# EmbarkStudios/kajiya

Hardware: NVIDIA H100
Metric: gi_rays_per_sec (higher is better)
Workload: dtype f32

## Files before the change

include/kjb_tlas.h:

```cpp
#ifndef KJB_TLAS_H
#define KJB_TLAS_H
#include "kjb.h"
#ifdef __cplusplus
extern "C" {
#endif
int kjb_tlas_download(kjb_context *ctx, uint32_t out_counts[3], int32_t *out_root, void *nodes, void *tris, void *tri_info, int32_t *parent);

#define KJB_TLAS_TRACE_ANY_HIT 1u
#define KJB_TLAS_TRACE_CULL_BACK 2u
#define KJB_TLAS_TRACE_BRUTE_FORCE 4u
int kjb_tlas_trace(kjb_context *ctx, const float *rays, uint32_t n, uint32_t flags, float *out);
#ifdef __cplusplus
}
#endif
#endif
```

kajiya_b200/_abi.py:

```python
import ctypes as C
import numpy as np

FMT = dict(R32_FLOAT=1, RG32_UINT=2, RGBA32_FLOAT=3, RGBA32_UINT=4, RGBA16_FLOAT=5, RG16_FLOAT=6, RGBA8_UNORM=7,
           RGBA8_SNORM=8, R8_UNORM=9, R8_SNORM=10, RGBA16_SNORM=11, A2R10G10B10_UNORM=12, R11G11B10_UFLOAT=13,
           R32_UINT=14, R16_FLOAT=15, RG32_FLOAT=16)
FMT_NAME = {v: k for k, v in FMT.items()}
FMT_NUMPY = {1: (np.float32, 1), 2: (np.uint32, 2), 3: (np.float32, 4), 4: (np.uint32, 4), 5: (np.float16, 4), 6: (np.float16, 2),
             7: (np.uint8, 4), 8: (np.int8, 4), 9: (np.uint8, 1), 10: (np.int8, 1), 11: (np.int16, 4), 12: (np.uint32, 1),
             13: (np.uint32, 1), 14: (np.uint32, 1), 15: (np.float16, 1), 16: (np.float32, 2)}


class Image(C.Structure):
    _fields_ = [("data", C.c_void_p), ("width", C.c_uint32), ("height", C.c_uint32), ("format", C.c_uint32), ("layers", C.c_uint32)]


class Buffer(C.Structure):
    _fields_ = [("data", C.c_void_p), ("size_bytes", C.c_uint64)]


class MeshMaterial(C.Structure):
    _fields_ = [("base_color_mult", C.c_float * 4), ("maps", C.c_uint32 * 4), ("roughness_mult", C.c_float), ("metalness_factor", C.c_float),
                ("emissive", C.c_float * 3), ("flags", C.c_uint32), ("map_transforms", C.c_float * 24)]


class TextureDesc(C.Structure):
    _fields_ = [("texels", C.c_void_p), ("width", C.c_uint32), ("height", C.c_uint32), ("mip_count", C.c_uint32), ("srgb", C.c_uint32)]


class WorldDesc(C.Structure):
    _fields_ = [("render_width", C.c_uint32), ("render_height", C.c_uint32), ("temporal_upscale_width", C.c_uint32), ("temporal_upscale_height", C.c_uint32),
                ("spatial_reuse_pass_count", C.c_uint32), ("use_raytraced_reservoir_visibility", C.c_uint32),
                ("enable_ircache", C.c_uint32), ("enable_rtr", C.c_uint32), ("enable_taa", C.c_uint32), ("tile_y0", C.c_uint32), ("tile_y1", C.c_uint32),
                ("tile_rank", C.c_uint32), ("tile_count", C.c_uint32), ("enable_ssao", C.c_uint32), ("enable_lighting", C.c_uint32), ("hard_sun", C.c_uint32)]


class MeshDesc(C.Structure):
    _fields_ = [("positions", C.c_void_p), ("normals", C.c_void_p), ("uvs", C.c_void_p), ("colors", C.c_void_p), ("material_ids", C.c_void_p),
                ("indices", C.c_void_p), ("vertex_count", C.c_uint32), ("index_count", C.c_uint32), ("materials", C.POINTER(MeshMaterial)),
                ("material_count", C.c_uint32), ("maps", C.POINTER(TextureDesc)), ("map_count", C.c_uint32), ("use_lights", C.c_uint32)]


class WorldFrame(C.Structure):
    _fields_ = [("camera_position", C.c_float * 3), ("camera_rotation", C.c_float * 4), ("vertical_fov_deg", C.c_float), ("near_plane", C.c_float),
                ("sun_direction", C.c_float * 3), ("delta_time_seconds", C.c_float),
                ("host_gbuffer", C.c_void_p), ("host_depth", C.c_void_p), ("host_geometric_normal", C.c_void_p), ("host_velocity", C.c_void_p),
                ("host_result", C.c_void_p), ("capture_slot", C.c_uint32), ("replay_slot", C.c_uint32), ("streaming", C.c_uint32)]


assert C.sizeof(MeshMaterial) == 152


class KjbError(RuntimeError):
    pass


class KjbLib:

    def __init__(self, path):
        self.path = path
        self.dll = C.CDLL(path, mode=C.RTLD_LOCAL)
        d = self.dll
        P = C.c_void_p
        sig = {
            "kjb_abi_version": (C.c_int, []),
            "kjb_backend_name": (C.c_char_p, []),
            "kjb_create": (C.c_int, [C.c_int, C.POINTER(P)]),
            "kjb_destroy": (None, [P]),
            "kjb_sync": (C.c_int, [P]),
            "kjb_last_error": (C.c_char_p, [P]),
            "kjb_launch_count": (C.c_uint64, [P]),
            "kjb_stream": (P, [P]),
            "kjb_format_texel_bytes": (C.c_uint32, [C.c_uint32]),
            "kjb_image_alloc": (C.c_int, [P, C.c_uint32, C.c_uint32, C.c_uint32, C.c_uint32, C.POINTER(Image)]),
            "kjb_image_free": (C.c_int, [P, C.POINTER(Image)]),
            "kjb_image_clear": (C.c_int, [P, C.POINTER(Image)]),
            "kjb_image_upload": (C.c_int, [P, C.POINTER(Image), P]),
            "kjb_image_download": (C.c_int, [P, C.POINTER(Image), P]),
            "kjb_ray_counters": (C.c_int, [P, C.POINTER(C.c_uint64 * 2), C.c_int]),
            "kjb_world_create": (C.c_int, [P, C.POINTER(WorldDesc), C.POINTER(P)]),
            "kjb_world_destroy": (None, [P]),
            "kjb_world_add_mesh": (C.c_int, [P, C.POINTER(MeshDesc), C.POINTER(C.c_uint32)]),
            "kjb_world_add_instance": (C.c_int, [P, C.c_uint32, C.POINTER(C.c_float * 12), C.POINTER(C.c_uint32)]),
            "kjb_world_set_instance_transform": (C.c_int, [P, C.c_uint32, C.POINTER(C.c_float * 12)]),
            "kjb_world_remove_instance": (C.c_int, [P, C.c_uint32]),
            "kjb_world_set_sun_size_multiplier": (C.c_int, [P, C.c_float]),
            "kjb_world_set_sun_color_multiplier": (C.c_int, [P, C.POINTER(C.c_float * 3)]),
            "kjb_world_set_sky_ambient": (C.c_int, [P, C.POINTER(C.c_float * 3)]),
            "kjb_world_set_render_overrides": (C.c_int, [P, C.c_uint32, C.c_float]),
            "kjb_world_set_debug_shading_mode": (C.c_int, [P, C.c_uint32]),
            "kjb_world_reset_reference_accumulation": (C.c_int, [P]),
            "kjb_world_set_instance_emissive_multiplier": (C.c_int, [P, C.c_uint32, C.c_float]),
            "kjb_world_set_blue_noise": (C.c_int, [P, P]),
            "kjb_world_set_spatial_resolve_offsets": (C.c_int, [P, P]),
            "kjb_world_render_frame": (C.c_int, [P, C.POINTER(WorldFrame)]),
            "kjb_world_render_reference": (C.c_int, [P, C.POINTER(WorldFrame), C.c_uint32]),
            "kjb_world_frame_index": (C.c_uint32, [P]),
            "kjb_world_wait": (C.c_int, [P]),
            "kjb_world_get_image": (C.c_int, [P, C.c_char_p, C.POINTER(Image)]),
            "kjb_world_image_names": (C.c_char_p, [P]),
            "kjb_world_last_frame_stats": (C.c_int, [P, C.POINTER(C.c_uint64 * 4)]),
            "kjb_world_set_stop_after": (C.c_int, [P, C.c_char_p]),
            "kjb_world_set_profiling": (C.c_int, [P, C.c_uint32]),
            "kjb_comm_nccl_unique_id": (C.c_int, [P]),
            "kjb_comm_init_nccl": (C.c_int, [P, P, C.c_uint32, C.c_uint32]),
            "kjb_comm_set_callback": (C.c_int, [P, P, P, C.c_uint32, C.c_uint32]),
            "kjb_world_pass_timings": (C.c_char_p, [P]),
            "kjb_set_debug_serial": (C.c_int, [P, C.c_uint32]),
            "kjb_tlas_stats": (C.c_int, [P, C.POINTER(C.c_uint64 * 2)]),
            "kjb_graph_stats": (C.c_int, [P, C.POINTER(C.c_uint64 * 2)]),
            "kjb_graph_select": (C.c_int, [P, C.c_uint32]), "kjb_set_pass_queue": (C.c_int, [P, C.c_uint32]), "kjb_async_passes_supported": (C.c_int, [P]),
            "kjb_world_set_cuda_graph": (C.c_int, [P, C.c_uint32]), "kjb_world_set_async_compute": (C.c_int, [P, C.c_uint32]),
            "kjb_set_option": (C.c_int, [P, C.c_uint32, C.c_uint32]),
            "kjb_timer_record": (C.c_int, [P, C.c_uint32]),
            "kjb_timer_elapsed_ms": (C.c_int, [P, C.c_uint32, C.c_uint32, C.POINTER(C.c_float)]),
        }
        self.missing = []
        for name, (res, args) in sig.items():
            try:
                fn = getattr(d, name)
            except AttributeError:
                self.missing.append(name)
                continue
            fn.restype = res
            fn.argtypes = args
        if self.missing:
            raise KjbError(f"{path} does not export: {self.missing}")
        if d.kjb_abi_version() != 1:
            raise KjbError("ABI version mismatch")
        self.has_tlas_download = hasattr(d, "kjb_tlas_download")
        if self.has_tlas_download:
            d.kjb_tlas_download.restype = C.c_int
            d.kjb_tlas_download.argtypes = [P, C.POINTER(C.c_uint32 * 3), C.POINTER(C.c_int32), P, P, P, P]
        self.has_tlas_trace = hasattr(d, "kjb_tlas_trace")
        if self.has_tlas_trace:
            d.kjb_tlas_trace.restype = C.c_int
            d.kjb_tlas_trace.argtypes = [P, P, C.c_uint32, C.c_uint32, P]

    @property
    def backend(self):
        return self.dll.kjb_backend_name().decode()


def declared_symbols(include_dir):
    import re, os
    names = []
    for h in ("kjb.h", "kjb_world.h"):
        src = open(os.path.join(include_dir, h)).read()
        names += re.findall(r"\b(kjb_[a-z0-9_]+)\s*\(", src)
    return sorted(set(names))
```

kajiya_b200/csrc/kjb_api.cu:

```cuda
#include "kjb_context.h"
#include "kjb_ircache.cuh"
#include "kjb_bvh_build.cuh"
#include "../../include/kjb_tlas.h"
#include <algorithm>

using namespace kjb;

KJB_DEV void box_of_tri(const float3 a, const float3 b, const float3 c, float* out6) {
    out6[0] = kjb_min(a.x, kjb_min(b.x, c.x)); out6[1] = kjb_min(a.y, kjb_min(b.y, c.y)); out6[2] = kjb_min(a.z, kjb_min(b.z, c.z));
    out6[3] = kjb_max(a.x, kjb_max(b.x, c.x)); out6[4] = kjb_max(a.y, kjb_max(b.y, c.y)); out6[5] = kjb_max(a.z, kjb_max(b.z, c.z));
}
KJB_KERNEL(256) k_refit_tris(SceneView sc, BvhTri* tris, float* tri_box, uint32_t slot_count, Rows kjb_rows) {
    const uint32_t s = blockIdx.x * blockDim.x + threadIdx.x;
    if (s >= slot_count) return;
    const uint32_t gid = tris[s].gid;
    if (gid >= sc.tri_count) return;
    const TriInfo ti = sc.tri_info[gid];
    const kjb_instance& inst = sc.instances[ti.instance];
    const kjb_gpu_mesh mesh = sc.meshes[inst.mesh_index];
    float3 wv[3];
    for (int k = 0; k < 3; ++k) {
        const uint32_t idx = vb_u32(sc, mesh.index_offset + (ti.prim * 3 + k) * 4);
        const float* v = reinterpret_cast<const float*>(sc.vertices + mesh.vertex_core_offset + size_t(idx) * 16);
        wv[k] = xform_point(inst.transform, f3(v[0], v[1], v[2]));
    }
    BvhTri t = tris[s];
    t.v0[0] = wv[0].x; t.v0[1] = wv[0].y; t.v0[2] = wv[0].z;
    t.e1[0] = wv[1].x - wv[0].x; t.e1[1] = wv[1].y - wv[0].y; t.e1[2] = wv[1].z - wv[0].z;
    t.e2[0] = wv[2].x - wv[0].x; t.e2[1] = wv[2].y - wv[0].y; t.e2[2] = wv[2].z - wv[0].z;
    tris[s] = t;
    box_of_tri(wv[0], wv[1], wv[2], tri_box + size_t(s) * 6);
}
KJB_KERNEL(256) k_refit_nodes(BvhNode* nodes, const int32_t* parent, uint32_t* count, float* slot_box, const float* tri_box, const uint32_t* node_count, Rows kjb_rows) {
    uint32_t i = blockIdx.x * blockDim.x + threadIdx.x;
    if (i >= *node_count) return;
    uint32_t leaves = 0;
    for (int k = 0; k < 2; ++k) {
        const int32_t ch = nodes[i].child[k];
        if (ch >= 0) continue;
        const uint32_t enc = uint32_t(~ch), first = enc >> 3, n = (enc & 7u) + 1u;
        float b[6] = {3.4e38f, 3.4e38f, 3.4e38f, -3.4e38f, -3.4e38f, -3.4e38f};
        for (uint32_t t = 0; t < n; ++t) for (int a = 0; a < 3; ++a) { b[a] = kjb_min(b[a], tri_box[size_t(first + t) * 6 + a]); b[3 + a] = kjb_max(b[3 + a], tri_box[size_t(first + t) * 6 + 3 + a]); }
        for (int a = 0; a < 6; ++a) slot_box[(size_t(i) * 2 + k) * 6 + a] = b[a];
        write_padded_slot(nodes[i], k, b);
        ++leaves;
    }
    if (leaves == 0) return;
    for (;;) {
#if defined(__CUDA_ARCH__)
        __threadfence();
#endif
        if (atom_add(&count[i], leaves) + leaves < 2u) return;
        const int32_t p = parent[i];
        if (p < 0) return;
        float u[6];
        for (int a = 0; a < 3; ++a) { u[a] = kjb_min(slot_box[(size_t(i) * 2) * 6 + a], slot_box[(size_t(i) * 2 + 1) * 6 + a]); u[3 + a] = kjb_max(slot_box[(size_t(i) * 2) * 6 + 3 + a], slot_box[(size_t(i) * 2 + 1) * 6 + 3 + a]); }
        const uint32_t pi = uint32_t(p >> 1); const int pk = p & 1;
        for (int a = 0; a < 6; ++a) slot_box[(size_t(pi) * 2 + pk) * 6 + a] = u[a];
        write_padded_slot(nodes[pi], pk, u);
        i = pi; leaves = 1;
    }
}

extern "C" {

int kjb_abi_version(void) { return KJB_ABI_VERSION; }
#if defined(KJB_EMU)
const char* kjb_backend_name(void) { return "emu-cpu"; }
#else
#if defined(KJB_FAST)
const char* kjb_backend_name(void) { return "cuda-sm90a-fast"; }
#else
const char* kjb_backend_name(void) { return "cuda-sm90a"; }
#endif
#endif

static thread_local std::string g_create_error;

int kjb_create(int device, kjb_context** out) {
    *out = nullptr;
#if !defined(KJB_EMU)
    int n = 0;
    if (cudaGetDeviceCount(&n) != cudaSuccess || n == 0) { g_create_error = "kjb_create: no CUDA device (this library has no CPU fallback)"; return 1; }
    if (device < 0 || device >= n) { g_create_error = "kjb_create: invalid device ordinal"; return 1; }
    if (cudaSetDevice(device) != cudaSuccess) { g_create_error = "kjb_create: cudaSetDevice failed"; return 1; }
#endif
    kjb_context* c = new kjb_context();
    c->device = device;
#if !defined(KJB_EMU)
    if (cudaStreamCreateWithFlags(&c->compute_stream, cudaStreamNonBlocking) != cudaSuccess) { delete c; g_create_error = "kjb_create: stream creation failed"; return 1; }
    c->stream = c->compute_stream;
#endif
    memset(&c->g, 0, sizeof(c->g));
    c->d_ray_counters = (unsigned long long*)dev_alloc(2 * sizeof(unsigned long long));
    c->g.scene.ray_counters = c->d_ray_counters;
    c->g.scene.root = ~int32_t(0);
    *out = c;
    return 0;
}
void kjb_destroy(kjb_context* c) {
    if (!c) return;
    dev_sync(c);
    dev_free(c->d_vertices); dev_free(c->d_meshes); dev_free(c->d_instances); dev_free(c->d_nodes); dev_free(c->d_tris); dev_free(c->d_tri_info);
    dev_free(c->d_node_parent); dev_free(c->d_refit_count); dev_free(c->d_slot_box); dev_free(c->d_tri_box); dev_free(c->d_bvh_scratch); dev_free(c->d_inst_prefix);
    dev_free(c->d_tex_data); dev_free(c->d_tex_desc); dev_free(c->d_lights); dev_free(c->d_ray_counters); dev_free(c->d_prev_instances); dev_free(c->d_resolve_offsets);
    for (auto& kv : c->ircache_scratch) { const auto& s = kv.second; dev_free(s.claim_rank); dev_free(s.claim_vertex); dev_free(s.life_pending); dev_free(s.scan); dev_free(s.claim_bits); dev_free(s.aux_prev); dev_free(s.entry_vertex); }
#if !defined(KJB_EMU)
    if (c->pinned_staging) cudaFreeHost(c->pinned_staging);
    for (auto& ge : c->graph_execs) if (ge) cudaGraphExecDestroy(ge);
    for (auto& ev : c->queue_events) if (ev) cudaEventDestroy(ev);
    for (auto& st : c->copy_streams) if (st) cudaStreamDestroy(st);
    if (c->compute_stream) cudaStreamDestroy(c->compute_stream);
#endif
    delete c;
}
int kjb_sync(kjb_context* c) {
    if (dev_sync(c)) return c->fail("kjb_sync: stream synchronize failed");
    const char* e = dev_check(c); if (e) return c->fail(std::string("kjb_sync: ") + e);
    return 0;
}
const char* kjb_last_error(kjb_context* c) { return c ? c->last_error.c_str() : g_create_error.c_str(); }
uint64_t kjb_launch_count(kjb_context* c) { return c->launches; }
#if defined(KJB_EMU)
void* kjb_stream(kjb_context* c) { return (void*)c->stream; }
#else
void* kjb_stream(kjb_context* c) { return (void*)c->compute_stream; }
#endif
uint32_t kjb_format_texel_bytes(uint32_t f) { return texel_bytes(f); }

int kjb_image_alloc(kjb_context* c, uint32_t w, uint32_t h, uint32_t layers, uint32_t fmt, kjb_image* out) {
    if (!texel_bytes(fmt) || !w || !h) return c->fail("kjb_image_alloc: bad format or extent");
    out->width = w; out->height = h; out->format = fmt; out->layers = layers ? layers : 1;
    out->data = dev_alloc(image_bytes(*out));
    return out->data ? 0 : c->fail("kjb_image_alloc: out of device memory");
}
static void drop_ircache_scratch(kjb_context* c, const void* p) {
    auto it = c->ircache_scratch.find(p);
    if (it == c->ircache_scratch.end()) return;
    dev_sync(c);
    const auto& s = it->second; dev_free(s.claim_rank); dev_free(s.claim_vertex); dev_free(s.life_pending); dev_free(s.scan); dev_free(s.claim_bits); dev_free(s.aux_prev); dev_free(s.entry_vertex);
    c->ircache_scratch.erase(it);
}
int kjb_image_free(kjb_context* c, kjb_image* img) {
    drop_ircache_scratch(c, img->data);
    dev_free(img->data); img->data = nullptr; return 0;
}
int kjb_image_clear(kjb_context* c, const kjb_image* img) { c->invalidate_positions(); return dev_memset(c, img->data, 0, image_bytes(*img)); }
int kjb_image_fill_u8(kjb_context* c, const kjb_image* img, uint32_t v) { c->invalidate_positions(); return dev_memset(c, img->data, int(v), image_bytes(*img)); }
int kjb_image_copy(kjb_context* c, const kjb_image* dst, const kjb_image* src) { c->invalidate_positions();
    if (image_bytes(*dst) != image_bytes(*src) || dst->format != src->format) return c->fail("kjb_image_copy: extent/format mismatch");
    return dev_d2d(c, dst->data, src->data, image_bytes(*dst));
}
int kjb_image_upload(kjb_context* c, const kjb_image* dst, const void* src) { c->invalidate_positions(); return dev_h2d(c, dst->data, src, image_bytes(*dst)); }
int kjb_image_download(kjb_context* c, const kjb_image* src, void* dst) { return dev_d2h(c, dst, src->data, image_bytes(*src)); }
#if defined(KJB_EMU)
int kjb_image_upload_on(kjb_context* c, uint32_t, const kjb_image* dst, const void* src) { return kjb_image_upload(c, dst, src); }
int kjb_image_download_on(kjb_context* c, uint32_t, const kjb_image* src, void* dst) { return kjb_image_download(c, src, dst); }
int kjb_image_upload_rows_on(kjb_context* c, uint32_t, const kjb_image* dst, const void* src, uint32_t r0, uint32_t n) {
    if (r0 + n > dst->height) return c->fail("kjb_image_upload_rows_on: rows out of range");
    const size_t rb = size_t(dst->width) * texel_bytes(dst->format); c->invalidate_positions(); memcpy((char*)dst->data + rb * r0, (const char*)src + rb * r0, rb * n); return 0; }
int kjb_image_download_rows_on(kjb_context* c, uint32_t, const kjb_image* src, void* dst, uint32_t r0, uint32_t n) {
    if (r0 + n > src->height) return c->fail("kjb_image_download_rows_on: rows out of range");
    const size_t rb = size_t(src->width) * texel_bytes(src->format); memcpy((char*)dst + rb * r0, (const char*)src->data + rb * r0, rb * n); return 0; }
int kjb_event_record(kjb_context*, uint32_t, uint32_t) { return 0; }
int kjb_queue_wait_event(kjb_context*, uint32_t, uint32_t) { return 0; }
int kjb_event_synchronize(kjb_context*, uint32_t) { return 0; }
#else
int kjb_image_upload_on(kjb_context* c, uint32_t q, const kjb_image* dst, const void* src) {
    c->invalidate_positions();
    cudaStream_t st = c->queue(q); if (!st) return c->fail("kjb_image_upload_on: bad queue");
    return cudaMemcpyAsync(dst->data, src, image_bytes(*dst), cudaMemcpyHostToDevice, st) != cudaSuccess ? c->fail("kjb_image_upload_on: copy failed") : 0;
}
int kjb_image_upload_rows_on(kjb_context* c, uint32_t q, const kjb_image* dst, const void* src, uint32_t r0, uint32_t n) {
    if (r0 + n > dst->height || (dst->layers > 1)) return c->fail("kjb_image_upload_rows_on: rows out of range");
    c->invalidate_positions();
    cudaStream_t st = c->queue(q); if (!st) return c->fail("kjb_image_upload_rows_on: bad queue");
    const size_t rb = size_t(dst->width) * texel_bytes(dst->format);
    return cudaMemcpyAsync((char*)dst->data + rb * r0, (const char*)src + rb * r0, rb * n, cudaMemcpyHostToDevice, st) != cudaSuccess ? c->fail("kjb_image_upload_rows_on: copy failed") : 0;
}
int kjb_image_download_rows_on(kjb_context* c, uint32_t q, const kjb_image* src, void* dst, uint32_t r0, uint32_t n) {
    if (r0 + n > src->height || (src->layers > 1)) return c->fail("kjb_image_download_rows_on: rows out of range");
    cudaStream_t st = c->queue(q); if (!st) return c->fail("kjb_image_download_rows_on: bad queue");
    const size_t rb = size_t(src->width) * texel_bytes(src->format);
    return cudaMemcpyAsync((char*)dst + rb * r0, (const char*)src->data + rb * r0, rb * n, cudaMemcpyDeviceToHost, st) != cudaSuccess ? c->fail("kjb_image_download_rows_on: copy failed") : 0;
}
int kjb_image_download_on(kjb_context* c, uint32_t q, const kjb_image* src, void* dst) {
    cudaStream_t st = c->queue(q); if (!st) return c->fail("kjb_image_download_on: bad queue");
    return cudaMemcpyAsync(dst, src->data, image_bytes(*src), cudaMemcpyDeviceToHost, st) != cudaSuccess ? c->fail("kjb_image_download_on: copy failed") : 0;
}
int kjb_event_record(kjb_context* c, uint32_t e, uint32_t q) {
    cudaStream_t st = c->queue(q); if (!st || e >= KJB_MAX_EVENTS) return c->fail("kjb_event_record: bad queue or event");
    if (!c->queue_events[e] && cudaEventCreateWithFlags(&c->queue_events[e], cudaEventDisableTiming) != cudaSuccess) return c->fail("kjb_event_record: cudaEventCreate failed");
    return cudaEventRecord(c->queue_events[e], st) != cudaSuccess ? c->fail("kjb_event_record: record failed") : 0;
}
int kjb_queue_wait_event(kjb_context* c, uint32_t q, uint32_t e) {
    cudaStream_t st = c->queue(q); if (!st || e >= KJB_MAX_EVENTS) return c->fail("kjb_queue_wait_event: bad queue or event");
    if (!c->queue_events[e]) return 0;
    return cudaStreamWaitEvent(st, c->queue_events[e], 0) != cudaSuccess ? c->fail("kjb_queue_wait_event: wait failed") : 0;
}
int kjb_event_synchronize(kjb_context* c, uint32_t e) {
    if (e >= KJB_MAX_EVENTS) return c->fail("kjb_event_synchronize: bad event");
    if (!c->queue_events[e]) return 0;
    return cudaEventSynchronize(c->queue_events[e]) != cudaSuccess ? c->fail("kjb_event_synchronize: failed") : 0;
}
#endif
int kjb_buffer_alloc(kjb_context* c, uint64_t n, kjb_buffer* out) { out->data = dev_alloc(n); out->size_bytes = n; return out->data ? 0 : c->fail("kjb_buffer_alloc: out of device memory"); }
int kjb_buffer_free(kjb_context* c, kjb_buffer* b) { drop_ircache_scratch(c, b->data); dev_free(b->data); b->data = nullptr; return 0; }
int kjb_buffer_upload(kjb_context* c, const kjb_buffer* dst, uint64_t off, const void* src, uint64_t n) { return dev_h2d(c, (char*)dst->data + off, src, n); }
int kjb_buffer_download(kjb_context* c, const kjb_buffer* src, uint64_t off, void* dst, uint64_t n) { return dev_d2h(c, dst, (const char*)src->data + off, n); }

int kjb_scene_set_geometry(kjb_context* c, const void* vb, uint64_t vb_bytes, const kjb_gpu_mesh* meshes, const uint32_t* counts, uint32_t n) {
    dev_sync(c);
    dev_free(c->d_vertices); dev_free(c->d_meshes);
    c->h_vertices.assign((const uint8_t*)vb, (const uint8_t*)vb + vb_bytes);
    c->h_meshes.assign(meshes, meshes + n); c->h_index_counts.assign(counts, counts + n);
    c->d_vertices = (uint8_t*)dev_alloc(vb_bytes); c->d_meshes = (kjb_gpu_mesh*)dev_alloc(n * sizeof(kjb_gpu_mesh));
    if (!c->d_vertices || !c->d_meshes) return c->fail("kjb_scene_set_geometry: out of device memory");
    dev_h2d(c, c->d_vertices, c->h_vertices.data(), vb_bytes); dev_h2d(c, c->d_meshes, c->h_meshes.data(), n * sizeof(kjb_gpu_mesh));
    c->g.scene.vertices = c->d_vertices; c->g.scene.meshes = c->d_meshes;
    c->tlas_valid = false;
    return dev_sync(c);
}
int kjb_scene_set_textures(kjb_context* c, const kjb_texture_desc* t, uint32_t n) {
    dev_sync(c);
    dev_free(c->d_tex_data); dev_free(c->d_tex_desc); c->d_tex_data = nullptr; c->d_tex_desc = nullptr;
    std::vector<uint8_t> data; std::vector<uint4> desc(n);
    for (uint32_t i = 0; i < n; ++i) {
        size_t bytes = 0; for (uint32_t m = 0; m < t[i].mip_count; ++m) bytes += size_t(t[i].width >> m ? t[i].width >> m : 1) * (t[i].height >> m ? t[i].height >> m : 1) * 4;
        desc[i] = u4(uint32_t(data.size()), t[i].width, t[i].height, t[i].mip_count | (t[i].srgb << 16));
        data.insert(data.end(), t[i].texels, t[i].texels + bytes);
        while (data.size() & 15) data.push_back(0);
    }
    c->tex_count = n;
    if (n) {
        c->d_tex_data = (uint8_t*)dev_alloc(data.size()); c->d_tex_desc = (uint4*)dev_alloc(n * sizeof(uint4));
        if (!c->d_tex_data || !c->d_tex_desc) return c->fail("kjb_scene_set_textures: out of device memory");
        dev_h2d(c, c->d_tex_data, data.data(), data.size()); dev_h2d(c, c->d_tex_desc, desc.data(), n * sizeof(uint4));
    }
    c->g.scene.tex_data = c->d_tex_data; c->g.scene.tex_desc = c->d_tex_desc; c->g.scene.tex_count = n;
    return dev_sync(c);
}

static void* staging_slot(kjb_context* c, size_t bytes) {
    if (c->pinned_bytes < bytes) {
#if !defined(KJB_EMU)
        dev_sync(c); if (c->pinned_staging) cudaFreeHost(c->pinned_staging);
        if (cudaMallocHost(&c->pinned_staging, bytes * 4) != cudaSuccess) { c->pinned_staging = nullptr; c->pinned_bytes = 0; return nullptr; }
#else
        free(c->pinned_staging); c->pinned_staging = malloc(bytes * 4);
#endif
        c->pinned_bytes = bytes;
    }
    return (char*)c->pinned_staging + size_t(c->staging_seq++ & 3u) * c->pinned_bytes;
}
static int reserve_tlas(kjb_context* c, uint32_t tris, uint32_t instances) {
    const bool grow_tris = tris > c->bvh_tri_cap || !c->d_bvh_scratch, grow_inst = instances + 1 > c->bvh_inst_cap || !c->d_instances;
    if (!grow_tris && !grow_inst) return 0;
    dev_sync(c);
    if (grow_inst) {
        const uint32_t cap = std::max(instances + 1, c->bvh_inst_cap * 2);
        dev_free(c->d_instances); dev_free(c->d_inst_prefix);
        c->d_instances = (kjb_instance*)dev_alloc(size_t(cap) * sizeof(kjb_instance)); c->d_inst_prefix = (uint32_t*)dev_alloc(size_t(cap + 1) * 4);
        c->bvh_inst_cap = cap;
        if (!c->d_instances || !c->d_inst_prefix) { c->bvh_inst_cap = 0; return c->fail("kjb_rebuild_tlas: out of device memory"); }
    }
    if (grow_tris) {
        const uint32_t cap = std::max(std::max(tris, 1u), c->bvh_tri_cap + c->bvh_tri_cap / 2);
        dev_free(c->d_nodes); dev_free(c->d_tris); dev_free(c->d_tri_info); dev_free(c->d_node_parent); dev_free(c->d_refit_count); dev_free(c->d_slot_box);
        dev_free(c->d_tri_box); dev_free(c->d_bvh_scratch);
        c->d_nodes = (BvhNode*)dev_alloc(size_t(cap) * sizeof(BvhNode)); c->d_tris = (BvhTri*)dev_alloc(size_t(cap) * sizeof(BvhTri));
        c->d_tri_info = (TriInfo*)dev_alloc(size_t(cap + 1) * sizeof(TriInfo)); c->d_node_parent = (int32_t*)dev_alloc(size_t(cap) * 4);
        c->d_refit_count = (uint32_t*)dev_alloc(size_t(cap) * 4); c->d_slot_box = (float*)dev_alloc(size_t(cap) * 12 * sizeof(float));
        c->d_tri_box = (float*)dev_alloc(size_t(cap) * 6 * sizeof(float)); c->d_bvh_scratch = dev_alloc(bvh_build_scratch_bytes(cap));
        c->bvh_tri_cap = cap;
        if (!c->d_nodes || !c->d_tris || !c->d_tri_info || !c->d_node_parent || !c->d_refit_count || !c->d_slot_box || !c->d_tri_box || !c->d_bvh_scratch) {
            c->bvh_tri_cap = 0; return c->fail("kjb_rebuild_tlas: out of device memory");
        }
        c->d_node_count = bvh_build_node_count(c);
    }
    return 0;
}

int kjb_rebuild_tlas(kjb_context* c, const kjb_instance* inst, uint32_t n) {
    if (c->tlas_valid && c->h_instances.size() == n && (n == 0 || memcmp(c->h_instances.data(), inst, n * sizeof(kjb_instance)) == 0)) return 0;
    {
        bool same_topology = c->tlas_valid && c->h_instances.size() == n && n > 0 && c->node_count > 0 && c->d_node_parent;
        for (uint32_t i = 0; same_topology && i < n; ++i) same_topology = c->h_instances[i].mesh_index == inst[i].mesh_index;
        if (same_topology) {
            kjb_instance* stage = (kjb_instance*)staging_slot(c, n * sizeof(kjb_instance));
            if (!stage) return c->fail("kjb_rebuild_tlas: pinned staging allocation failed");
            memcpy(stage, inst, n * sizeof(kjb_instance));
            c->h_instances.assign(inst, inst + n);
            if (dev_h2d(c, c->d_instances, stage, n * sizeof(kjb_instance))) return c->fail("kjb_rebuild_tlas: instance upload failed");
            dev_memset(c, c->d_refit_count, 0, c->node_count * sizeof(uint32_t));
            const kjb::Rows kjb__rows = {0, 1};
            KJB_LAUNCH(c, k_refit_tris, KJB_DIMS(dim3((c->slot_count + 255) / 256), dim3(256)), c->g.scene, c->d_tris, c->d_tri_box, c->slot_count);
            KJB_LAUNCH(c, k_refit_nodes, KJB_DIMS(dim3((c->node_count + 255) / 256), dim3(256)), c->d_nodes, (const int32_t*)c->d_node_parent, c->d_refit_count, c->d_slot_box, (const float*)c->d_tri_box, (const uint32_t*)c->d_node_count);
            c->tlas_refits++;
            KJB_PASS_EPILOGUE(c, "rebuild tlas (refit)");
        }
    }
    uint64_t total = 0;
    for (uint32_t i = 0; i < n; ++i) {
        if (inst[i].mesh_index >= c->h_meshes.size()) return c->fail("kjb_rebuild_tlas: instance references an unknown mesh");
        total += c->h_index_counts[inst[i].mesh_index] / 3;
    }
    if (total >= (1u << 28)) return c->fail("kjb_rebuild_tlas: more than 2^28 triangles (leaf references hold 28 bits of triangle slot)");
    const uint32_t ntri = uint32_t(total);
    if (reserve_tlas(c, ntri, n)) return 1;
    const size_t inst_bytes = size_t(n) * sizeof(kjb_instance), stage_bytes = inst_bytes + size_t(n + 1) * 4;
    uint8_t* stage = (uint8_t*)staging_slot(c, stage_bytes);
    if (!stage) return c->fail("kjb_rebuild_tlas: pinned staging allocation failed");
    memcpy(stage, inst, inst_bytes);
    uint32_t* prefix = (uint32_t*)(stage + inst_bytes);
    prefix[0] = 0;
    for (uint32_t i = 0; i < n; ++i) prefix[i + 1] = prefix[i] + c->h_index_counts[inst[i].mesh_index] / 3;
    if ((n && dev_h2d(c, c->d_instances, stage, inst_bytes)) || dev_h2d(c, c->d_inst_prefix, prefix, size_t(n + 1) * 4)) return c->fail("kjb_rebuild_tlas: instance upload failed");
    c->tlas_rebuilds++;
    c->h_instances.assign(inst, inst + n);
    c->g.scene.nodes = c->d_nodes; c->g.scene.tris = c->d_tris; c->g.scene.tri_info = c->d_tri_info; c->g.scene.instances = c->d_instances;
    c->g.scene.tri_count = ntri;
    c->g.scene.root = ntri == 0 ? ~int32_t(0) : (ntri <= 4 ? ~int32_t(ntri - 1) : 0);
    c->slot_count = ntri ? ntri : 1;
    c->node_count = ntri > 4 ? ntri - 1 : 0;
    c->tlas_valid = true;
    if (ntri == 0) {
        if (dev_memset(c, c->d_tris, 0, sizeof(BvhTri))) return c->fail("kjb_rebuild_tlas: memset failed");
        KJB_PASS_EPILOGUE(c, "rebuild tlas");
    }
    if (bvh_build_on_device(c, n, ntri)) return 1;
    const kjb::Rows kjb__rows = {0, 1};
    KJB_LAUNCH(c, k_refit_tris, KJB_DIMS(dim3((ntri + 255) / 256), dim3(256)), c->g.scene, c->d_tris, c->d_tri_box, ntri);
    KJB_PASS_EPILOGUE(c, "rebuild tlas");
}

int kjb_tlas_download(kjb_context* c, uint32_t out_counts[3], int32_t* out_root, void* nodes, void* tris, void* tri_info, int32_t* parent) {
    if (dev_sync(c)) return c->fail("kjb_tlas_download: sync failed");
    uint32_t nodes_n = 0;
    if (c->tlas_valid && c->node_count) dev_d2h(c, &nodes_n, c->d_node_count, 4);
    if (dev_sync(c)) return c->fail("kjb_tlas_download: sync failed");
    const uint32_t slots = c->tlas_valid ? c->slot_count : 0, infos = c->tlas_valid ? c->g.scene.tri_count : 0;
    out_counts[0] = nodes_n; out_counts[1] = slots; out_counts[2] = infos;
    if (out_root) *out_root = c->g.scene.root;
    if (nodes && nodes_n) dev_d2h(c, nodes, c->d_nodes, size_t(nodes_n) * sizeof(BvhNode));
    if (parent && nodes_n) dev_d2h(c, parent, c->d_node_parent, size_t(nodes_n) * 4);
    if (tris && slots) dev_d2h(c, tris, c->d_tris, size_t(slots) * sizeof(BvhTri));
    if (tri_info && infos) dev_d2h(c, tri_info, c->d_tri_info, size_t(infos) * sizeof(TriInfo));
    if (dev_sync(c)) return c->fail("kjb_tlas_download: sync failed");
    const char* e = dev_check(c); if (e) return c->fail(std::string("kjb_tlas_download: ") + e);
    return 0;
}

}
KJB_KERNEL(128) k_tlas_trace(SceneView sc, const float* rays, uint32_t n, uint32_t flags, uint32_t slots, uint32_t* out, Rows kjb_rows) {
    const uint32_t i = blockIdx.x * blockDim.x + threadIdx.x;
    if (i >= n) return;
    const float* p = rays + size_t(i) * 8;
    Ray r; r.origin = f3(p[0], p[1], p[2]); r.tmin = p[3]; r.dir = f3(p[4], p[5], p[6]); r.tmax = p[7];
    const bool any = flags & KJB_TLAS_TRACE_ANY_HIT, cull = flags & KJB_TLAS_TRACE_CULL_BACK;
    HitInfo h; h.hit = false; h.t = r.tmax; h.u = 0; h.v = 0; h.gid = 0xffffffffu;
    if (flags & KJB_TLAS_TRACE_BRUTE_FORCE) {
        if (any) h.hit = intersect_leaf<true>(sc.tris, 0, slots, r, cull, h);
        else intersect_leaf<false>(sc.tris, 0, slots, r, cull, h);
    } else {
        h = any ? trace<true>(sc, r, cull) : trace<false>(sc, r, cull);
    }
    uint32_t* o = out + size_t(i) * 4;
    if (!h.hit) { o[0] = 0; o[1] = 0; o[2] = 0; o[3] = 0xffffffffu; }
    else if (any) { o[0] = 0; o[1] = 0; o[2] = 0; o[3] = 0; }
    else { o[0] = kjb_f2u(h.t); o[1] = kjb_f2u(h.u); o[2] = kjb_f2u(h.v); o[3] = h.gid; }
}
extern "C" {

int kjb_tlas_trace(kjb_context* c, const float* rays, uint32_t n, uint32_t flags, float* out) {
    if (!c->tlas_valid) return c->fail("kjb_tlas_trace: no acceleration structure (render a frame or call kjb_rebuild_tlas first)");
    if (flags & ~(KJB_TLAS_TRACE_ANY_HIT | KJB_TLAS_TRACE_CULL_BACK | KJB_TLAS_TRACE_BRUTE_FORCE)) return c->fail("kjb_tlas_trace: unknown flags");
    if (n == 0) return 0;
    if (dev_sync(c)) return c->fail("kjb_tlas_trace: sync failed");
    float* d_rays = (float*)dev_alloc(size_t(n) * 8 * sizeof(float));
    uint32_t* d_out = (uint32_t*)dev_alloc(size_t(n) * 4 * sizeof(uint32_t));
    int rc = 0;
    if (!d_rays || !d_out) rc = c->fail("kjb_tlas_trace: out of device memory");
    if (!rc && dev_h2d(c, d_rays, rays, size_t(n) * 8 * sizeof(float))) rc = c->fail("kjb_tlas_trace: upload failed");
    if (!rc) {
        const kjb::Rows kjb__rows = {0, 1};
        KJB_LAUNCH(c, k_tlas_trace, KJB_DIMS(dim3((n + 127) / 128), dim3(128)), c->g.scene, (const float*)d_rays, n, flags, c->slot_count, d_out);
        if (dev_d2h(c, out, d_out, size_t(n) * 4 * sizeof(uint32_t))) rc = c->fail("kjb_tlas_trace: download failed");
    }
    if (dev_sync(c) && !rc) rc = c->fail("kjb_tlas_trace: sync failed");
    const char* e = dev_check(c);
    if (e && !rc) rc = c->fail(std::string("kjb_tlas_trace: ") + e);
    dev_free(d_rays); dev_free(d_out);
    return rc;
}

#if defined(KJB_EMU)
int kjb_graph_begin(kjb_context*) { return 0; }
int kjb_graph_end(kjb_context*) { return 0; }
int kjb_graph_select(kjb_context*, uint32_t slot) { return slot < 4 ? 0 : 1; }
int kjb_set_pass_queue(kjb_context* c, uint32_t q) { return q == KJB_QUEUE_COMPUTE ? 0 : c->fail("kjb_set_pass_queue: this backend has one pass queue"); }
int kjb_async_passes_supported(kjb_context*) { return 0; }
#else
int kjb_graph_begin(kjb_context* c) {
    if (c->graph_capturing) return c->fail("kjb_graph_begin: already recording");
    if (cudaStreamBeginCapture(c->compute_stream, cudaStreamCaptureModeRelaxed) != cudaSuccess) { cudaGetLastError(); return c->fail("kjb_graph_begin: cudaStreamBeginCapture failed"); }
    c->graph_capturing = true;
    return 0;
}
int kjb_graph_end(kjb_context* c) {
    if (!c->graph_capturing) return c->fail("kjb_graph_end: not recording");
    cudaGraph_t g = nullptr;
    const cudaError_t e = cudaStreamEndCapture(c->compute_stream, &g);
    c->graph_capturing = false;
    if (e != cudaSuccess || !g) { cudaGetLastError(); return c->fail(std::string("kjb_graph_end: the recording was invalidated (") + cudaGetErrorString(e) + "): a pass inside the pair synchronised or touched another queue"); }
    cudaGraphExec_t& exec = c->graph_execs[c->graph_slot];
    if (exec) {
        cudaGraphExecUpdateResultInfo info;
        if (cudaGraphExecUpdate(exec, g, &info) != cudaSuccess) { cudaGetLastError(); cudaGraphExecDestroy(exec); exec = nullptr; }
    }
    if (!exec) {
        if (cudaGraphInstantiate(&exec, g, 0) != cudaSuccess) { cudaGetLastError(); cudaGraphDestroy(g); exec = nullptr; return c->fail("kjb_graph_end: cudaGraphInstantiate failed"); }
        c->graph_instantiations++;
    }
    const cudaError_t le = cudaGraphLaunch(exec, c->compute_stream);
    cudaGraphDestroy(g);
    if (le != cudaSuccess) return c->fail(std::string("kjb_graph_end: cudaGraphLaunch failed: ") + cudaGetErrorString(le));
    c->graph_launches++;
    return 0;
}
int kjb_graph_select(kjb_context* c, uint32_t slot) {
    if (slot >= 4) return c->fail("kjb_graph_select: 4 instances are kept");
    if (c->graph_capturing) return c->fail("kjb_graph_select: a recording is open");
    c->graph_slot = slot; return 0;
}
int kjb_set_pass_queue(kjb_context* c, uint32_t q) {
    if (q != KJB_QUEUE_COMPUTE && q != KJB_QUEUE_ASYNC) return c->fail("kjb_set_pass_queue: passes run on the compute or the async queue");
    if (q == KJB_QUEUE_ASYNC && c->debug_serial) return c->fail("kjb_set_pass_queue: serialised debugging keeps every pass on the compute queue");
    cudaStream_t st = c->queue(q); if (!st) return c->fail("kjb_set_pass_queue: queue creation failed");
    c->stream = st; return 0;
}
int kjb_async_passes_supported(kjb_context* c) { return c->debug_serial ? 0 : 1; }
#endif
int kjb_graph_stats(kjb_context* c, uint64_t out[2]) { out[0] = c->graph_launches; out[1] = c->graph_instantiations; return 0; }
int kjb_tlas_stats(kjb_context* c, uint64_t out[2]) { out[0] = c->tlas_rebuilds; out[1] = c->tlas_refits; return 0; }
int kjb_set_frame_constants(kjb_context* c, const kjb_frame_constants* fc, const kjb_triangle_light* lights, uint32_t n) {
    if (fc->triangle_light_count != n) return c->fail("kjb_set_frame_constants: triangle_light_count mismatch");
    c->g.fc = *fc; c->invalidate_positions();
    const float3 sc = sun_color_in_direction(*fc, sun_direction(*fc));
    c->g.sun_color[0] = sc.x; c->g.sun_color[1] = sc.y; c->g.sun_color[2] = sc.z; c->g.sun_color[3] = 0;
    if (n > c->lights_capacity) { dev_sync(c); dev_free(c->d_lights); c->d_lights = (kjb_triangle_light*)dev_alloc(n * sizeof(kjb_triangle_light)); c->lights_capacity = n; }
    if (n) {
        dev_h2d(c, c->d_lights, lights, n * sizeof(kjb_triangle_light)); dev_sync(c);
    }
    c->g.lights = c->d_lights;
    return 0;
}
int kjb_set_scissor(kjb_context* c, uint32_t y0, uint32_t y1) { c->scissor_y0 = y0; c->scissor_y1 = y1; return 0; }
static bool ordered_cache_has_run(const kjb_context* c) { return !c->ircache_scratch.empty(); }
int kjb_set_debug_serial(kjb_context* c, uint32_t on) {
    if (on && !c->debug_serial && ordered_cache_has_run(c)) return c->fail("kjb_set_debug_serial: the irradiance cache already runs on the ordered schedule; switch before its first frame");
    c->debug_serial = on != 0; return 0;
}
int kjb_set_option(kjb_context* c, uint32_t option, uint32_t value) {
    if (option == KJB_OPTION_HALF_RES_POSITION_CACHE) { c->opt_position_cache = value != 0; c->invalidate_positions(); return 0; }
    if (option == KJB_OPTION_ORDERED_CACHE_SCHEDULE) {
        if (!value && c->ordered_cache && ordered_cache_has_run(c)) return c->fail("kjb_set_option: the irradiance cache already runs on the ordered schedule; switch before its first frame");
        c->ordered_cache = value != 0; return 0;
    }
    return c->fail("kjb_set_option: unknown option");
}
int kjb_set_luts(kjb_context* c, const kjb_image* fg, const kjb_image* bn) {
    if (!check_img(c, *fg, KJB_FMT_RGBA16_FLOAT, "kjb_set_luts", "brdf_fg_lut", 64, 64)) return 1;
    if (!check_img(c, *bn, KJB_FMT_RGBA8_UNORM, "kjb_set_luts", "blue_noise", 256, 256)) return 1;
    c->g.brdf_fg_lut = img_ro(*fg); c->g.blue_noise = img_ro(*bn);
    return 0;
}
#if defined(KJB_EMU)
}
#include <chrono>
static std::chrono::steady_clock::time_point g_timer_slots[1024];
extern "C" {
int kjb_timer_record(kjb_context*, uint32_t slot) { if (slot >= 1024) return 1; g_timer_slots[slot] = std::chrono::steady_clock::now(); return 0; }
int kjb_timer_elapsed_ms(kjb_context*, uint32_t a, uint32_t b, float* out) { if (a >= 1024 || b >= 1024) return 1; *out = std::chrono::duration<float, std::milli>(g_timer_slots[b] - g_timer_slots[a]).count(); return 0; }
#else
int kjb_timer_record(kjb_context* c, uint32_t slot) {
    if (slot >= 1024) return c->fail("kjb_timer_record: slot out of range");
    if (c->timer_events.size() <= slot) c->timer_events.resize(slot + 1, nullptr);
    if (!c->timer_events[slot] && cudaEventCreate(&c->timer_events[slot]) != cudaSuccess) return c->fail("kjb_timer_record: cudaEventCreate failed");
    return cudaEventRecord(c->timer_events[slot], c->compute_stream) != cudaSuccess;
}
int kjb_timer_elapsed_ms(kjb_context* c, uint32_t a, uint32_t b, float* out) {
    if (a >= c->timer_events.size() || b >= c->timer_events.size() || !c->timer_events[a] || !c->timer_events[b]) return c->fail("kjb_timer_elapsed_ms: slot was never recorded");
    if (cudaEventSynchronize(c->timer_events[b]) != cudaSuccess) return c->fail("kjb_timer_elapsed_ms: event sync failed");
    return cudaEventElapsedTime(out, c->timer_events[a], c->timer_events[b]) != cudaSuccess;
}
#endif
int kjb_ray_counters(kjb_context* c, uint64_t out[2], int reset) {
    unsigned long long v[2] = {0, 0};
    dev_d2h(c, v, c->d_ray_counters, sizeof(v));
    if (dev_sync(c)) return c->fail("kjb_ray_counters: sync failed");
    out[0] = v[0]; out[1] = v[1];
    if (reset) dev_memset(c, c->d_ray_counters, 0, sizeof(v));
    return 0;
}

}
```

kajiya_b200/csrc/kjb_bvh.h:

```cpp
#pragma once
#include <stdint.h>

namespace kjb {

struct BvhNode { float n0[4], n1[4], n2[4]; int32_t child[4]; };
struct BvhTri { float v0[3]; uint32_t gid; float e1[3]; uint32_t pad0; float e2[3]; uint32_t pad1; };
struct TriInfo { uint32_t instance, prim; };

}
```

kajiya_b200/csrc/kjb_context.h:

```cpp
#pragma once
#include "kjb_trace.cuh"
#include "kjb_tile.cuh"
#include <map>
#include <initializer_list>
#include <string>
#include <vector>
#include <cstdio>
#include <cstring>
#include <cstdlib>

#if defined(KJB_EMU)
typedef void* kjb_stream_t;
#else
#include <cuda_runtime.h>
typedef cudaStream_t kjb_stream_t;
#endif

struct kjb_context {
    int device = 0;
    kjb_stream_t stream = nullptr;
    std::string last_error;
    uint64_t launches = 0;

    uint8_t* d_vertices = nullptr; size_t vertices_bytes = 0;
    kjb_gpu_mesh* d_meshes = nullptr;
    std::vector<uint8_t> h_vertices; std::vector<kjb_gpu_mesh> h_meshes; std::vector<uint32_t> h_index_counts;
    kjb_instance* d_instances = nullptr; std::vector<kjb_instance> h_instances; bool tlas_valid = false;
    kjb::BvhNode* d_nodes = nullptr; kjb::BvhTri* d_tris = nullptr; kjb::TriInfo* d_tri_info = nullptr;
    int32_t* d_node_parent = nullptr; uint32_t* d_refit_count = nullptr; float* d_slot_box = nullptr; float* d_tri_box = nullptr; uint32_t node_count = 0, slot_count = 0;
    uint64_t tlas_refits = 0, tlas_rebuilds = 0;
    uint32_t bvh_tri_cap = 0, bvh_inst_cap = 0; void* d_bvh_scratch = nullptr; uint32_t* d_inst_prefix = nullptr; uint32_t* d_node_count = nullptr;
    uint64_t staging_seq = 0;
    uint8_t* d_tex_data = nullptr; uint4* d_tex_desc = nullptr; uint32_t tex_count = 0;
    kjb_triangle_light* d_lights = nullptr; uint32_t lights_capacity = 0;
    unsigned long long* d_ray_counters = nullptr;
    void* pinned_staging = nullptr; size_t pinned_bytes = 0;
    kjb_instance* d_prev_instances = nullptr; uint32_t prev_instances_capacity = 0; std::vector<kjb_instance> h_prev_instances;
    int32_t* d_resolve_offsets = nullptr; std::vector<int32_t> h_resolve_offsets;
#if !defined(KJB_EMU)
    std::vector<cudaEvent_t> timer_events;
    cudaStream_t copy_streams[4] = {nullptr, nullptr, nullptr, nullptr};
    cudaStream_t compute_stream = nullptr;
    cudaEvent_t queue_events[64] = {};
    cudaStream_t queue(uint32_t q) {
        if (q == 0) return compute_stream;
        if (q > 4) return nullptr;
        if (!copy_streams[q - 1]) {
            int lo = 0, hi = 0; cudaDeviceGetStreamPriorityRange(&lo, &hi);
            if (cudaStreamCreateWithPriority(&copy_streams[q - 1], cudaStreamNonBlocking, q == 4 ? hi : lo) != cudaSuccess) return nullptr;
        }
        return copy_streams[q - 1];
    }
#endif

#if !defined(KJB_EMU)
    cudaGraphExec_t graph_execs[4] = {nullptr, nullptr, nullptr, nullptr}; uint32_t graph_slot = 0; bool graph_capturing = false;
#endif
    uint64_t graph_launches = 0, graph_instantiations = 0;
    kjb::Globals g;
    struct IrcacheScratch { void* claim_rank; void* claim_vertex; void* life_pending; void* scan; void* claim_bits; void* aux_prev; void* entry_vertex; };
    std::map<const void*, IrcacheScratch> ircache_scratch;

    kjb_allgather_fn ag_fn = nullptr; void* ag_user = nullptr; uint32_t rank = 0, nranks = 1; void* nccl_comm = nullptr;

    uint32_t scissor_y0 = 0, scissor_y1 = 0;
    struct PosCache { float4* d = nullptr; size_t cap = 0; const void* src = nullptr; uint32_t w = 0, h = 0; float gts[4] = {0, 0, 0, 0}; uint64_t epoch = ~0ull; };
    PosCache pos_a, pos_b; uint64_t epoch_a = 0, epoch_b = 0; bool opt_position_cache = false;
    void invalidate_positions() { epoch_a++; epoch_b++; }
    bool debug_serial = false;
#if defined(KJB_EMU)
    bool ordered_cache = false;
#else
    bool ordered_cache = true;
#endif
    kjb::Rows rows_for(uint32_t H) const {
        kjb::Rows r; r.y0 = 0; r.y1 = int(H);
        if (scissor_y1 > scissor_y0) { r.y0 = int(scissor_y0 < H ? scissor_y0 : H); r.y1 = int(scissor_y1 < H ? scissor_y1 : H); }
        return r;
    }

    int fail(const std::string& msg) { last_error = msg; return 1; }
};

namespace kjb {

#if defined(KJB_EMU)
inline void* dev_alloc(size_t n) { return calloc(n ? n : 1, 1); }
inline void dev_free(void* p) { free(p); }
inline int dev_h2d(kjb_context*, void* d, const void* h, size_t n) { memcpy(d, h, n); return 0; }
inline int dev_d2h(kjb_context*, void* h, const void* d, size_t n) { memcpy(h, d, n); return 0; }
inline int dev_d2d(kjb_context*, void* d, const void* s, size_t n) { memcpy(d, s, n); return 0; }
inline int dev_memset(kjb_context*, void* d, int v, size_t n) { memset(d, v, n); return 0; }
inline int dev_sync(kjb_context*) { return 0; }
inline const char* dev_check(kjb_context*) { return nullptr; }
#else
inline void* dev_alloc(size_t n) {
    void* p = nullptr;
    if (cudaMalloc(&p, n ? n : 1) != cudaSuccess) return nullptr;
    static thread_local cudaStream_t setup = nullptr;
    if (!setup && cudaStreamCreateWithFlags(&setup, cudaStreamNonBlocking) != cudaSuccess) { setup = nullptr; cudaFree(p); return nullptr; }
    if (cudaMemsetAsync(p, 0, n ? n : 1, setup) != cudaSuccess || cudaStreamSynchronize(setup) != cudaSuccess) { cudaFree(p); return nullptr; }
    return p;
}
inline void dev_free(void* p) { if (p) cudaFree(p); }
inline int dev_h2d(kjb_context* c, void* d, const void* h, size_t n) { return cudaMemcpyAsync(d, h, n, cudaMemcpyHostToDevice, c->stream) != cudaSuccess; }
inline int dev_d2h(kjb_context* c, void* h, const void* d, size_t n) { return cudaMemcpyAsync(h, d, n, cudaMemcpyDeviceToHost, c->stream) != cudaSuccess; }
inline int dev_d2d(kjb_context* c, void* d, const void* s, size_t n) { return cudaMemcpyAsync(d, s, n, cudaMemcpyDeviceToDevice, c->stream) != cudaSuccess; }
inline int dev_memset(kjb_context* c, void* d, int v, size_t n) { return cudaMemsetAsync(d, v, n, c->stream) != cudaSuccess; }
inline int dev_sync(kjb_context* c) {
    int rc = cudaStreamSynchronize(c->compute_stream) != cudaSuccess;
    for (cudaStream_t st : c->copy_streams) if (st) rc |= cudaStreamSynchronize(st) != cudaSuccess;
    return rc;
}
inline const char* dev_check(kjb_context*) { cudaError_t e = cudaGetLastError(); return e == cudaSuccess ? nullptr : cudaGetErrorString(e); }
#endif

inline uint32_t texel_bytes(uint32_t f) {
    switch (f) {
        case KJB_FMT_R32_FLOAT: case KJB_FMT_RG16_FLOAT: case KJB_FMT_RGBA8_UNORM: case KJB_FMT_RGBA8_SNORM:
        case KJB_FMT_A2R10G10B10_UNORM: case KJB_FMT_R11G11B10_UFLOAT: case KJB_FMT_R32_UINT: return 4;
        case KJB_FMT_RG32_UINT: case KJB_FMT_RGBA16_FLOAT: case KJB_FMT_RGBA16_SNORM: case KJB_FMT_RG32_FLOAT: return 8;
        case KJB_FMT_RGBA32_FLOAT: case KJB_FMT_RGBA32_UINT: return 16;
        case KJB_FMT_R8_UNORM: case KJB_FMT_R8_SNORM: return 1;
        case KJB_FMT_R16_FLOAT: return 2;
        default: return 0;
    }
}
inline size_t image_bytes(const kjb_image& i) { return size_t(i.width) * i.height * (i.layers ? i.layers : 1) * texel_bytes(i.format); }

inline int tile_mode(std::initializer_list<const kjb_image*> imgs) {
#if defined(KJB_EMU)
    (void)imgs; return KJB_TILE_LOADS;
#else
    for (const kjb_image* i : imgs)
        if (!texel_bytes(i->format) || uint64_t(i->width) * texel_bytes(i->format) % 16 || uintptr_t(i->data) % 16 || i->layers > 1) return KJB_TILE_LOADS;
    return KJB_TILE_ROWS;
#endif
}

inline bool check_img(kjb_context* c, const kjb_image& i, uint32_t fmt, const char* pass, const char* name, uint32_t w = 0, uint32_t h = 0) {
    if (!i.data) { c->fail(std::string(pass) + ": image '" + name + "' is null"); return false; }
    if (i.format != fmt) { c->fail(std::string(pass) + ": image '" + name + "' has format " + std::to_string(i.format) + ", expected " + std::to_string(fmt)); return false; }
    if (w && (i.width != w || i.height != h)) { c->fail(std::string(pass) + ": image '" + name + "' has the wrong extent"); return false; }
    return true;
}

}

#if defined(KJB_EMU)
#define KJB_KERNEL(bounds) static void
#define KJB_KERNEL_OCC(bounds, min_blocks) static void
#define KJB_LAUNCH(ctx, kernel, dims, ...) do { if (kjb__rows.y1 > kjb__rows.y0) { kjb_emu::launch(dims, [&]() { kernel(__VA_ARGS__, kjb__rows); }); (ctx)->launches++; } } while (0)
#define KJB_LAUNCH_SYNC(ctx, kernel, dims, ...) do { if (kjb__rows.y1 > kjb__rows.y0) { kjb_emu::launch_sync(dims, [&]() { kernel(__VA_ARGS__, kjb__rows); }); (ctx)->launches++; } } while (0)
#define KJB_LAUNCH_ORDERED(ctx, kernel, dims, ...) do { if (kjb__rows.y1 > kjb__rows.y0) { kjb_emu::g_serial++; kjb_emu::launch(dims, [&]() { kernel(__VA_ARGS__, kjb__rows); }); kjb_emu::g_serial--; (ctx)->launches++; } } while (0)
#else
#define KJB_KERNEL(bounds) __global__ void __launch_bounds__(bounds)
#define KJB_KERNEL_OCC(bounds, min_blocks) __global__ void __launch_bounds__(bounds, min_blocks)
#define KJB_LAUNCH(ctx, kernel, dims, ...) do { if (kjb__rows.y1 > kjb__rows.y0) { kernel<<<dims, 0, (ctx)->stream>>>(__VA_ARGS__, kjb__rows); (ctx)->launches++; } } while (0)
#define KJB_LAUNCH_SYNC KJB_LAUNCH
#define KJB_LAUNCH_ORDERED KJB_LAUNCH
#endif
#define KJB_DIMS(...) __VA_ARGS__
#ifndef KJB_RAY_BX
#define KJB_RAY_BX 8
#endif
#ifndef KJB_RAY_BY
#define KJB_RAY_BY 16
#endif
#define KJB_ROWS(ctx, H) const kjb::Rows kjb__rows = (ctx)->rows_for(H)
#define KJB_GRID2D(W, H, BX, BY) dim3(((W) + (BX) - 1) / (BX), (unsigned(kjb__rows.y1 - kjb__rows.y0) + (BY) - 1) / (BY), 1), dim3((BX), (BY), 1)
#define KJB_PX int x = int(blockIdx.x * blockDim.x + threadIdx.x), y = kjb_rows.y0 + int(blockIdx.y * blockDim.y + threadIdx.y); if (y >= kjb_rows.y1) return

#define KJB_PIXELS(SERIAL, W, H, ...) do { \
        if constexpr (SERIAL) { \
            if (blockIdx.x | blockIdx.y | threadIdx.x | threadIdx.y) return; \
            for (int by = kjb_rows.y0; by < kjb_rows.y1; by += KJB_RAY_BY) for (int bx = 0; bx < (W); bx += KJB_RAY_BX) \
                for (int y = by; y < by + KJB_RAY_BY && y < kjb_rows.y1 && y < (H); ++y) for (int x = bx; x < bx + KJB_RAY_BX && x < (W); ++x) { __VA_ARGS__; } \
        } else { KJB_PX; if (x >= (W) || y >= (H)) return; __VA_ARGS__; } } while (0)
#define KJB_SERIAL_1D(n, ...) do { if (blockIdx.x | threadIdx.x) return; for (uint32_t i = 0, n__ = (n); i < n__; ++i) { __VA_ARGS__; } } while (0)
#define KJB_LAUNCH_CACHE(ctx, bound, kernel, dims, ...) do { \
        if ((bound) && (ctx)->debug_serial) KJB_LAUNCH(ctx, kernel<true>, KJB_DIMS(dim3(1), dim3(32)), __VA_ARGS__); \
        else if (bound) KJB_LAUNCH_ORDERED(ctx, kernel<false>, KJB_DIMS(dims), __VA_ARGS__); \
        else KJB_LAUNCH(ctx, kernel<false>, KJB_DIMS(dims), __VA_ARGS__); } while (0)
// ... 3 lines not shown
```

kajiya_b200/csrc/kjb_device.cuh:

```cuda
#pragma once
#include "../../include/kjb_numeric.h"
#include "../../include/kjb.h"

#if defined(__CUDACC__)
#define KJB_DEV __host__ __device__ __forceinline__
#else
#define KJB_DEV inline
#endif

namespace kjb {

KJB_DEV float2 f2(float x, float y) { float2 r; r.x = x; r.y = y; return r; }
KJB_DEV float2 f2(float a) { return f2(a, a); }
KJB_DEV float3 f3(float x, float y, float z) { float3 r; r.x = x; r.y = y; r.z = z; return r; }
KJB_DEV float3 f3(float a) { return f3(a, a, a); }
KJB_DEV float4 f4(float x, float y, float z, float w) { float4 r; r.x = x; r.y = y; r.z = z; r.w = w; return r; }
KJB_DEV float4 f4(float a) { return f4(a, a, a, a); }
KJB_DEV float4 f4(float3 v, float w) { return f4(v.x, v.y, v.z, w); }
KJB_DEV float3 xyz(float4 v) { return f3(v.x, v.y, v.z); }
KJB_DEV float2 xy(float4 v) { return f2(v.x, v.y); }
KJB_DEV float2 xy(float3 v) { return f2(v.x, v.y); }
KJB_DEV int2 i2(int x, int y) { int2 r; r.x = x; r.y = y; return r; }
KJB_DEV uint2 u2(uint32_t x, uint32_t y) { uint2 r; r.x = x; r.y = y; return r; }
KJB_DEV uint4 u4(uint32_t x, uint32_t y, uint32_t z, uint32_t w) { uint4 r; r.x = x; r.y = y; r.z = z; r.w = w; return r; }
// ... 195 lines not shown
KJB_DEV float4 working_to_linear(float4 v) {
    return f4(ycbcr_to_rgb(xyz(v) * v.x), v.w);
}

struct StreamState { float p_q_sel, M_sum; };
struct Reservoir {
    float w_sum; uint32_t payload; float M, W;
    KJB_DEV static Reservoir create() { Reservoir r; r.w_sum = 0; r.payload = 0; r.M = 0; r.W = 0; return r; }
    KJB_DEV static Reservoir from_raw(uint2 raw) { Reservoir r; r.w_sum = 0; r.payload = raw.x; const float2 mw = unpack_2x16f(raw.y); r.M = mw.x; r.W = mw.y; return r; }
    KJB_DEV uint2 as_raw() const { return u2(payload, pack_2x16f(M, kjb_max(0.0f, W))); }
    KJB_DEV bool update(float w, uint32_t sample_payload, uint32_t& rng) {
        w_sum += w; M += 1;
        const float dart = rand01(rng);
        const float prob = w / w_sum;
        if (prob >= dart) { payload = sample_payload; return true; }
        return false;
    }
    KJB_DEV bool update_with_stream(const Reservoir& r, float p_q, float weight, StreamState& st, uint32_t sample_payload, uint32_t& rng) {
        st.M_sum += r.M;
        if (update(p_q * weight * r.W * r.M, sample_payload, rng)) { st.p_q_sel = p_q; return true; }
        return false;
    }
    KJB_DEV void init_with_stream(float p_q, float weight, StreamState& st, uint32_t sample_payload) {
        payload = sample_payload; w_sum = p_q * weight; M = (weight != 0) ? 1.0f : 0.0f; W = weight;
        st.p_q_sel = p_q; st.M_sum = M;
    }
    KJB_DEV void finish_stream(const StreamState& st) { M = st.M_sum; W = w_sum / kjb_max(1e-8f, M * st.p_q_sel); }
};

struct Img { const uint8_t* p; int w, h; };
struct ImgW { uint8_t* p; int w, h; };
KJB_DEV Img img_ro(const kjb_image& i) { Img r; r.p = (const uint8_t*)i.data; r.w = int(i.width); r.h = int(i.height); return r; }
KJB_DEV ImgW img_rw(const kjb_image& i) { ImgW r; r.p = (uint8_t*)i.data; r.w = int(i.width); r.h = int(i.height); return r; }
KJB_DEV Img as_ro(const ImgW& i) { Img r; r.p = i.p; r.w = i.w; r.h = i.h; return r; }
KJB_DEV bool inb(const Img& i, int x, int y) { return (unsigned)x < (unsigned)i.w && (unsigned)y < (unsigned)i.h; }
KJB_DEV bool inb(const ImgW& i, int x, int y) { return (unsigned)x < (unsigned)i.w && (unsigned)y < (unsigned)i.h; }
KJB_DEV size_t texel_offset(int w, int h, int x, int y, int layer, size_t texel_bytes) {
    const uint32_t in_layer = uint32_t(y) * uint32_t(w) + uint32_t(x);
    return (layer == 0 ? size_t(in_layer) : size_t(layer) * size_t(uint32_t(h) * uint32_t(w)) + in_layer) * texel_bytes;
}
template <typename T> KJB_DEV T ld_raw(const Img& i, int x, int y, int layer = 0) { return *(const T*)(i.p + texel_offset(i.w, i.h, x, y, layer, sizeof(T))); }
template <typename T> KJB_DEV void st_raw(const ImgW& i, int x, int y, T v, int layer = 0) { *(T*)(i.p + texel_offset(i.w, i.h, x, y, layer, sizeof(T))) = v; }
KJB_DEV float4 half4_to_float4(uint2 v) { return f4(kjb_f16_to_f32(v.x & 0xffffu), kjb_f16_to_f32(v.x >> 16), kjb_f16_to_f32(v.y & 0xffffu), kjb_f16_to_f32(v.y >> 16)); }
KJB_DEV uint2 float4_to_half4(float4 v) { return u2(pack_2x16f(v.x, v.y), pack_2x16f(v.z, v.w)); }
KJB_DEV float snorm8(uint32_t b) { return kjb_max(KJB_DIV_INT_CONST(float(int(int8_t(b & 0xffu))), 127.0f), -1.0f); }
KJB_DEV float snorm16(uint32_t b) { return kjb_max(KJB_DIV_INT_CONST(float(int(int16_t(b & 0xffffu))), 32767.0f), -1.0f); }
KJB_DEV uint32_t enc_unorm(float v, float scale) { return uint32_t(kjb_clamp(v, 0.0f, 1.0f) * scale + 0.5f); }
KJB_DEV int enc_snorm(float v, float scale) { v = kjb_clamp(v, -1.0f, 1.0f) * scale; return v >= 0.0f ? int(v + 0.5f) : -int(-v + 0.5f); }

KJB_DEV float  ld_r32f(const Img& i, int x, int y) { return inb(i, x, y) ? ld_raw<float>(i, x, y) : 0.0f; }
KJB_DEV float4 ld_rgba32f(const Img& i, int x, int y) { return inb(i, x, y) ? ld_raw<float4>(i, x, y) : f4(0.0f); }
KJB_DEV uint4  ld_rgba32u(const Img& i, int x, int y) { return inb(i, x, y) ? ld_raw<uint4>(i, x, y) : u4(0, 0, 0, 0); }
KJB_DEV uint2  ld_rg32u(const Img& i, int x, int y) { return inb(i, x, y) ? ld_raw<uint2>(i, x, y) : u2(0, 0); }
KJB_DEV float4 ld_rgba16f(const Img& i, int x, int y, int layer = 0) { return inb(i, x, y) ? half4_to_float4(ld_raw<uint2>(i, x, y, layer)) : f4(0.0f); }
KJB_DEV float2 ld_rg16f(const Img& i, int x, int y) { return inb(i, x, y) ? unpack_2x16f(ld_raw<uint32_t>(i, x, y)) : f2(0.0f); }
KJB_DEV float4 ld_rgba8u(const Img& i, int x, int y) {
    if (!inb(i, x, y)) return f4(0.0f);
    const uint32_t v = ld_raw<uint32_t>(i, x, y);
    return f4(KJB_DIV_INT_CONST(float(v & 255u), 255.0f), KJB_DIV_INT_CONST(float((v >> 8) & 255u), 255.0f), KJB_DIV_INT_CONST(float((v >> 16) & 255u), 255.0f), KJB_DIV_INT_CONST(float(v >> 24), 255.0f));
}
KJB_DEV float4 ld_rgba8s(const Img& i, int x, int y) {
    if (!inb(i, x, y)) return f4(0.0f);
    const uint32_t v = ld_raw<uint32_t>(i, x, y);
    return f4(snorm8(v), snorm8(v >> 8), snorm8(v >> 16), snorm8(v >> 24));
}
KJB_DEV float ld_r8u(const Img& i, int x, int y) { return inb(i, x, y) ? KJB_DIV_INT_CONST(float(ld_raw<uint8_t>(i, x, y)), 255.0f) : 0.0f; }
KJB_DEV float ld_r8s(const Img& i, int x, int y) { return inb(i, x, y) ? snorm8(ld_raw<uint8_t>(i, x, y)) : 0.0f; }
KJB_DEV float4 ld_rgba16s(const Img& i, int x, int y) {
    if (!inb(i, x, y)) return f4(0.0f);
    const uint2 v = ld_raw<uint2>(i, x, y);
    return f4(snorm16(v.x), snorm16(v.x >> 16), snorm16(v.y), snorm16(v.y >> 16));
}
KJB_DEV float3 ld_a2r10g10b10(const Img& i, int x, int y) {
    if (!inb(i, x, y)) return f3(0.0f);
    const uint32_t v = ld_raw<uint32_t>(i, x, y);
    return f3(KJB_DIV_INT_CONST(float((v >> 20) & 1023u), 1023.0f), KJB_DIV_INT_CONST(float((v >> 10) & 1023u), 1023.0f), KJB_DIV_INT_CONST(float(v & 1023u), 1023.0f));
}
KJB_DEV void st_r32f(const ImgW& i, int x, int y, float v) { if (inb(i, x, y)) st_raw<float>(i, x, y, v); }
KJB_DEV void st_rgba32f(const ImgW& i, int x, int y, float4 v) { if (inb(i, x, y)) st_raw<float4>(i, x, y, v); }
KJB_DEV void st_rgba32u(const ImgW& i, int x, int y, uint4 v) { if (inb(i, x, y)) st_raw<uint4>(i, x, y, v); }
KJB_DEV void st_rg32u(const ImgW& i, int x, int y, uint2 v) { if (inb(i, x, y)) st_raw<uint2>(i, x, y, v); }
KJB_DEV void st_rgba16f(const ImgW& i, int x, int y, float4 v, int layer = 0) { if (inb(i, x, y)) st_raw<uint2>(i, x, y, float4_to_half4(v), layer); }
KJB_DEV void st_rg16f(const ImgW& i, int x, int y, float a, float b) { if (inb(i, x, y)) st_raw<uint32_t>(i, x, y, pack_2x16f(a, b)); }
KJB_DEV void st_rgba8u(const ImgW& i, int x, int y, float4 v) {
    if (inb(i, x, y)) st_raw<uint32_t>(i, x, y, enc_unorm(v.x, 255.0f) | (enc_unorm(v.y, 255.0f) << 8) | (enc_unorm(v.z, 255.0f) << 16) | (enc_unorm(v.w, 255.0f) << 24));
}
KJB_DEV void st_rgba8s(const ImgW& i, int x, int y, float4 v) {
    if (inb(i, x, y)) st_raw<uint32_t>(i, x, y, (uint32_t(enc_snorm(v.x, 127.0f)) & 255u) | ((uint32_t(enc_snorm(v.y, 127.0f)) & 255u) << 8)
                                                    | ((uint32_t(enc_snorm(v.z, 127.0f)) & 255u) << 16) | ((uint32_t(enc_snorm(v.w, 127.0f)) & 255u) << 24));
}
KJB_DEV void st_r8u(const ImgW& i, int x, int y, float v) { if (inb(i, x, y)) st_raw<uint8_t>(i, x, y, uint8_t(enc_unorm(v, 255.0f))); }
KJB_DEV void st_r8s(const ImgW& i, int x, int y, float v) { if (inb(i, x, y)) st_raw<uint8_t>(i, x, y, uint8_t(enc_snorm(v, 127.0f))); }
KJB_DEV void st_rgba16s(const ImgW& i, int x, int y, float4 v) {
    if (inb(i, x, y)) st_raw<uint2>(i, x, y, u2((uint32_t(enc_snorm(v.x, 32767.0f)) & 0xffffu) | (uint32_t(enc_snorm(v.y, 32767.0f)) << 16),
                                                 (uint32_t(enc_snorm(v.z, 32767.0f)) & 0xffffu) | (uint32_t(enc_snorm(v.w, 32767.0f)) << 16)));
}
KJB_DEV void st_a2r10g10b10(const ImgW& i, int x, int y, float3 v) {
    if (inb(i, x, y)) st_raw<uint32_t>(i, x, y, (enc_unorm(v.x, 1023.0f) << 20) | (enc_unorm(v.y, 1023.0f) << 10) | enc_unorm(v.z, 1023.0f));
}
KJB_DEV uint32_t f32_to_uf(float v, int mant_bits) {
    if (!(v > 0.0f)) return 0u;
    const uint32_t u = kjb_f2u(v);
    const int e = int(u >> 23) - 127 + 15;
    const uint32_t m = (u & 0x7fffffu) >> (23 - mant_bits);
    if (e >= 31) return (30u << mant_bits) | ((1u << mant_bits) - 1u);
    if (e <= 0) {
        if (e < -mant_bits) return 0u;
        return ((u & 0x7fffffu) | 0x800000u) >> (23 - mant_bits + 1 - e);
    }
    return (uint32_t(e) << mant_bits) | m;
}
KJB_DEV float uf_to_f32(uint32_t v, int mant_bits) {
    const uint32_t e = v >> mant_bits, m = v & ((1u << mant_bits) - 1u);
    if (e == 0) return float(m) * kjb_exp2(float(-14 - mant_bits));
    if (e == 31) return kjb_u2f(0x7f800000u);
    return kjb_u2f(((e + 112u) << 23) | (m << (23 - mant_bits)));
}
KJB_DEV float3 ld_r11g11b10(const Img& i, int x, int y) {
    if (!inb(i, x, y)) return f3(0.0f);
    const uint32_t v = ld_raw<uint32_t>(i, x, y);
    return f3(uf_to_f32(v & 2047u, 6), uf_to_f32((v >> 11) & 2047u, 6), uf_to_f32(v >> 22, 5));
}
KJB_DEV void st_r11g11b10(const ImgW& i, int x, int y, float3 c) { if (inb(i, x, y)) st_raw<uint32_t>(i, x, y, f32_to_uf(c.x, 6) | (f32_to_uf(c.y, 6) << 11) | (f32_to_uf(c.z, 5) << 22)); }
KJB_DEV float ld_r16f(const Img& i, int x, int y) { return inb(i, x, y) ? kjb_f16_to_f32(ld_raw<uint16_t>(i, x, y)) : 0.0f; }
KJB_DEV void st_r16f(const ImgW& i, int x, int y, float v) { if (inb(i, x, y)) st_raw<uint16_t>(i, x, y, uint16_t(kjb_f32_to_f16(v))); }
KJB_DEV uint32_t ld_r32u(const Img& i, int x, int y) { return inb(i, x, y) ? ld_raw<uint32_t>(i, x, y) : 0u; }
KJB_DEV void st_r32u(const ImgW& i, int x, int y, uint32_t v) { if (inb(i, x, y)) st_raw<uint32_t>(i, x, y, v); }
KJB_DEV int clampi(int v, int n) { return v < 0 ? 0 : (v >= n ? n - 1 : v); }
KJB_DEV int2 nearest_clamp_px(const Img& i, float2 uv) {
    return i2(clampi(kjb_cvt_i32(kjb_floor(uv.x * float(i.w))), i.w), clampi(kjb_cvt_i32(kjb_floor(uv.y * float(i.h))), i.h));
}
template <typename F> KJB_DEV float4 bilinear_clamp(int w, int h, float2 uv, F fetch) {
    const float fx = uv.x * float(w) - 0.5f, fy = uv.y * float(h) - 0.5f;
    const float x0f = kjb_floor(fx), y0f = kjb_floor(fy);
    const float tx = fx - x0f, ty = fy - y0f;
    const int x0 = clampi(kjb_cvt_i32(x0f), w), x1 = clampi(kjb_cvt_i32(x0f) + 1, w), y0 = clampi(kjb_cvt_i32(y0f), h), y1 = clampi(kjb_cvt_i32(y0f) + 1, h);
    const float4 a = fetch(x0, y0), b = fetch(x1, y0), c = fetch(x0, y1), d = fetch(x1, y1);
    const float4 top = vlerp(a, b, tx), bot = vlerp(c, d, tx);
    return vlerp(top, bot, ty);
}
KJB_DEV float4 sample_cube_rgba16f(const Img& cube, float3 dir) {
    const float ax = kjb_abs(dir.x), ay = kjb_abs(dir.y), az = kjb_abs(dir.z);
    int face; float sc, tc, ma;
    if (ax >= ay && ax >= az) { ma = ax; if (dir.x >= 0) { face = 0; sc = -dir.z; tc = -dir.y; } else { face = 1; sc = dir.z; tc = -dir.y; } }
    else if (ay >= az) { ma = ay; if (dir.y >= 0) { face = 2; sc = dir.x; tc = dir.z; } else { face = 3; sc = dir.x; tc = -dir.z; } }
    else { ma = az; if (dir.z >= 0) { face = 4; sc = dir.x; tc = -dir.y; } else { face = 5; sc = -dir.x; tc = -dir.y; } }
    const float2 uv = f2(0.5f * (sc / ma + 1.0f), 0.5f * (tc / ma + 1.0f));
    return bilinear_clamp(cube.w, cube.h, uv, [&](int x, int y) { return ld_rgba16f(cube, x, y, face); });
}

struct Rows { int y0, y1; };

struct BvhNode;
struct BvhTri;
struct TriInfo;
struct SceneView {
    const BvhNode* nodes; const BvhTri* tris; const TriInfo* tri_info;
    const uint8_t* vertices; const kjb_gpu_mesh* meshes; const kjb_instance* instances;
    const uint8_t* tex_data; const uint4* tex_desc;
    uint32_t tex_count, tri_count;
    int32_t root;
    unsigned long long* ray_counters;
};
struct Globals {
    kjb_frame_constants fc;
    float sun_color[4];
    const kjb_triangle_light* lights;
    Img brdf_fg_lut;
    Img blue_noise;
    SceneView scene;
};

struct ViewRayContext {
    float4 ray_dir_ws_h, ray_origin_ws_h, ray_hit_cs, ray_hit_vs_h, ray_hit_ws_h;
    KJB_DEV float3 ray_dir_ws() const { return normalize(xyz(ray_dir_ws_h)); }
    KJB_DEV float3 ray_origin_ws() const { return xyz(ray_origin_ws_h) / ray_origin_ws_h.w; }
    KJB_DEV float3 ray_hit_vs() const { return xyz(ray_hit_vs_h) / ray_hit_vs_h.w; }
    KJB_DEV float3 ray_hit_ws() const { return xyz(ray_hit_ws_h) / ray_hit_ws_h.w; }
    KJB_DEV float3 biased_secondary_ray_origin_ws() const { return ray_hit_ws() - ray_dir_ws() * (length(ray_hit_vs()) + length(ray_hit_ws())) * 1e-4f; }
    KJB_DEV float3 biased_secondary_ray_origin_ws_with_normal(float3 normal) const {
        const float3 hw = ray_hit_ws();
        const float3 ws_abs = vabs(hw);
        const float max_comp = kjb_max(kjb_max(ws_abs.x, ws_abs.y), kjb_max(ws_abs.z, -ray_hit_vs().z));
        return hw + (normal - ray_dir_ws()) * kjb_max(1e-4f, max_comp * 1e-6f);
    }
    KJB_DEV static ViewRayContext from_uv(const kjb_view_constants& vc, float2 uv) {
        ViewRayContext r;
        const float2 cs = uv_to_cs(uv);
        r.ray_dir_ws_h = mul(vc.view_to_world, mul(vc.sample_to_view, f4(cs.x, cs.y, 0.0f, 1.0f)));
        r.ray_origin_ws_h = mul(vc.view_to_world, mul(vc.sample_to_view, f4(cs.x, cs.y, 1.0f, 1.0f)));
        r.ray_hit_cs = f4(0.0f); r.ray_hit_vs_h = f4(0.0f); r.ray_hit_ws_h = f4(0.0f);
        return r;
    }
    KJB_DEV static ViewRayContext from_uv_and_depth(const kjb_view_constants& vc, float2 uv, float depth) {
        ViewRayContext r = from_uv(vc, uv);
        const float2 cs = uv_to_cs(uv);
        r.ray_hit_cs = f4(cs.x, cs.y, depth, 1.0f);
        r.ray_hit_vs_h = mul(vc.sample_to_view, r.ray_hit_cs);
        r.ray_hit_ws_h = mul(vc.view_to_world, r.ray_hit_vs_h);
        return r;
    }
    KJB_DEV static ViewRayContext from_uv_and_biased_depth(const kjb_view_constants& vc, float2 uv, float depth) {
        return from_uv_and_depth(vc, uv, kjb_min(1.0f, depth * kjb_u2f(0x3f800040u)));
    }
};
KJB_DEV float3 hit_ws_from_uv_depth(const kjb_view_constants& vc, float2 uv, float depth) {
    const float2 cs = uv_to_cs(uv);
    const float4 h = mul(vc.view_to_world, mul(vc.sample_to_view, f4(cs.x, cs.y, depth, 1.0f)));
    return xyz(h) / h.w;
}
KJB_DEV float3 hit_vs_from_uv_depth(const kjb_view_constants& vc, float2 uv, float depth) {
    const float2 cs = uv_to_cs(uv);
    const float4 h = mul(vc.sample_to_view, f4(cs.x, cs.y, depth, 1.0f));
    return xyz(h) / h.w;
}
KJB_DEV float3 get_eye_position(const kjb_view_constants& vc) { const float4 e = mul(vc.view_to_world, f4(0, 0, 0, 1)); return xyz(e) / e.w; }
KJB_DEV float3 direction_view_to_world(const kjb_view_constants& vc, float3 v) { return xyz(mul(vc.view_to_world, f4(v, 0))); }
KJB_DEV float3 direction_world_to_view(const kjb_view_constants& vc, float3 v) { return xyz(mul(vc.world_to_view, f4(v, 0))); }
KJB_DEV float3 position_world_to_clip(const kjb_view_constants& vc, float3 v) { const float4 p = mul(vc.view_to_clip, mul(vc.world_to_view, f4(v, 1))); return xyz(p) / p.w; }
KJB_DEV float3 position_world_to_sample(const kjb_view_constants& vc, float3 v) { const float4 p = mul(vc.view_to_sample, mul(vc.world_to_view, f4(v, 1))); return xyz(p) / p.w; }
KJB_DEV float pixel_cone_spread_angle_from_image_height(const kjb_view_constants& vc, float image_height) { return kjb_atan(2.0f * vc.clip_to_view.m[0] / image_height); }
KJB_DEV int2 halfres_subsample_offset(uint32_t frame_index) {
    const uint32_t i = frame_index & 3u;
    return i2(i < 2u ? 1 : 0, (i == 0u || i == 3u) ? 1 : 0);
}
struct RayCone { float width, spread_angle; };
KJB_DEV RayCone ray_cone_propagate(RayCone c, float surface_spread_angle, float hit_t) { RayCone r; r.width = c.spread_angle * hit_t + c.width; r.spread_angle = c.spread_angle + surface_spread_angle; return r; }

KJB_DEV float4 blue_noise_for_pixel(const Globals& g, uint32_t px, uint32_t py, uint32_t n) {
    const float2 r2 = r2_sequence(n);
    const uint32_t ox = kjb_cvt_u32(r2.x * 256.0f), oy = kjb_cvt_u32(r2.y * 256.0f);
    return ld_rgba8u(g.blue_noise, int((px + ox) & 255u), int((py + oy) & 255u)) * 255.0f / 256.0f + 0.5f / 256.0f;
}

KJB_DEV float2 atm_sphere_intersection(float3 ray_start, float3 ray_dir, float3 center, float radius) {
    ray_start = ray_start - center;
    const float a = dot(ray_dir, ray_dir);
    const float b = 2.0f * dot(ray_start, ray_dir);
    const float c = dot(ray_start, ray_start) - (radius * radius);
    float d = b * b - 4 * a * c;
    if (d < 0) return f2(-1.0f);
    d = kjb_sqrt(d);
    return f2(-b - d, -b + d) / (2 * a);
}
#define KJB_PLANET_RADIUS 6371000.0f
#define KJB_ATMOSPHERE_HEIGHT 100000.0f
KJB_DEV float3 atm_density(float3 pos_ws) {
    const float h = length(pos_ws - f3(0, -KJB_PLANET_RADIUS, 0)) - KJB_PLANET_RADIUS;
    return f3(kjb_exp(-kjb_max(0.0f, h / (KJB_ATMOSPHERE_HEIGHT * 0.08f))), kjb_exp(-kjb_max(0.0f, h / (KJB_ATMOSPHERE_HEIGHT * 0.012f))),
              kjb_max(0.0f, 1 - kjb_abs(h - 25000.0f) / 15000.0f));
}
KJB_DEV float3 atm_integrate_optical_depth(float3 ray_start, float3 ray_dir) {
    const float2 isect = atm_sphere_intersection(ray_start, ray_dir, f3(0, -KJB_PLANET_RADIUS, 0), KJB_PLANET_RADIUS + KJB_ATMOSPHERE_HEIGHT);
    const float step_size = isect.y / 8.0f;
    float3 od = f3(0.0f);
    for (int i = 0; i < 8; i++) od += atm_density(ray_start + ray_dir * (float(i) + 0.5f) * step_size) * step_size;
    return od;
}
KJB_DEV float3 atm_absorb(float3 od) {
    const float3 cr = f3(5.802f, 13.558f, 33.100f) * 1e-6f, cm = f3(3.996f, 3.996f, 3.996f) * 1e-6f, co = f3(0.650f, 1.881f, 0.085f) * 1e-6f;
    return vexp(-(od.x * cr + od.y * cm * 1.1f + od.z * co) * 1.0f);
}
KJB_DEV float3 atm_integrate_scattering(float3 ray_start, float3 ray_dir, float ray_length, float3 light_dir) {
    const float2 isect = atm_sphere_intersection(ray_start, ray_dir, f3(0, -KJB_PLANET_RADIUS, 0), KJB_PLANET_RADIUS + KJB_ATMOSPHERE_HEIGHT);
    ray_length = kjb_min(ray_length, isect.y);
    if (isect.x > 0) { ray_start = ray_start + ray_dir * isect.x; ray_length -= isect.x; }
    const float costh = dot(ray_dir, light_dir);
    const float phase_r = 3 * (1 + costh * costh) / (16 * 3.14159265359f);
    const float gk = 1.55f * 0.85f - 0.55f * 0.85f * 0.85f * 0.85f;
    const float kc = gk * costh;
    const float phase_m = (1 - gk * gk) / ((4 * 3.14159265359f) * (1 - kc) * (1 - kc));
    float3 od = f3(0.0f), rayleigh = f3(0.0f), mie = f3(0.0f);
    float prev_t = 0;
    for (int i = 1; i <= 16; i++) {
        const float t = kjb_pow(float(i) / 16.0f, 5.0f) * ray_length;
        const float step_size = t - prev_t;
        const float3 pos = ray_start + ray_dir * kjb_lerp(prev_t, t, 0.5f);
        const float3 dens = atm_density(pos);
        od += dens * step_size;
        const float3 view_tr = atm_absorb(od);
        const float3 light_tr = atm_absorb(atm_integrate_optical_depth(pos, light_dir));
        rayleigh += view_tr * light_tr * phase_r * dens.x * step_size;
        mie += view_tr * light_tr * phase_m * dens.y * step_size;
        prev_t = t;
    }
    const float3 cr = f3(5.802f, 13.558f, 33.100f) * 1e-6f, cm = f3(3.996f, 3.996f, 3.996f) * 1e-6f;
    return (rayleigh * cr + mie * cm) * f3(1.0f) * 20.0f;
}
KJB_DEV float3 sun_direction(const kjb_frame_constants& fc) { return f3(fc.sun_direction[0], fc.sun_direction[1], fc.sun_direction[2]); }
KJB_DEV float3 atmosphere_default(const kjb_frame_constants& fc, float3 wi, float3 light_dir) {
    const float3 amb = f3(fc.sky_ambient[0], fc.sky_ambient[1], fc.sky_ambient[2]), mult = f3(fc.sun_color_multiplier[0], fc.sun_color_multiplier[1], fc.sun_color_multiplier[2]);
    return (amb + mult * atm_integrate_scattering(f3(0.0f), wi, kjb_u2f(0x7f800000u), light_dir)) * fc.pre_exposure;
}
KJB_DEV float3 sun_color_in_direction(const kjb_frame_constants& fc, float3 dir) {
    const float3 mult = f3(fc.sun_color_multiplier[0], fc.sun_color_multiplier[1], fc.sun_color_multiplier[2]);
    return 20.0f * mult * fc.pre_exposure * atm_absorb(atm_integrate_optical_depth(f3(0.0f), dir));
}
KJB_DEV float3 sample_sun_direction(const kjb_frame_constants& fc, float2 urand, bool soft) {
    if (soft && fc.sun_angular_radius_cos < 1.0f) {
        const float3x3 basis = build_orthonormal_basis(normalize(sun_direction(fc)));
        return mul(basis, uniform_sample_cone(urand, fc.sun_angular_radius_cos));
    }
    return sun_direction(fc);
}

struct BrdfValue { float3 value_over_pdf, value; float pdf; float3 transmission_fraction; };
struct BrdfSample { float3 value_over_pdf, value; float pdf; float3 transmission_fraction; float3 wi; float approx_roughness; };
KJB_DEV BrdfValue brdf_value_invalid() { BrdfValue r; r.value_over_pdf = f3(0.0f); r.value = f3(0.0f); r.pdf = 0; r.transmission_fraction = f3(0.0f); return r; }
KJB_DEV BrdfSample brdf_sample_invalid() { BrdfSample r; r.value_over_pdf = f3(0.0f); r.value = f3(0.0f); r.pdf = 0; r.transmission_fraction = f3(0.0f); r.wi = f3(0, 0, -1); r.approx_roughness = 0; return r; }
KJB_DEV float3 fresnel_schlick(float3 f0, float3 f90, float cos_theta) { return vlerp(f0, f90, kjb_pow(kjb_max(0.0f, 1.0f - cos_theta), 5.0f)); }
// ... 144 lines not shown
```

kajiya_b200/csrc/kjb_passes_ircache.cu:

```cuda
#include "kjb_context.h"
#include "kjb_ircache.cuh"

using namespace kjb;

#define MAX_ENTRIES KJB_IRCACHE_MAX_ENTRIES

KJB_DEV uint32_t tid1d() { return blockIdx.x * blockDim.x + threadIdx.x; }

KJB_DEV bool ircache_slot_is_stale_duplicate(const uint32_t* indirection, uint32_t alloc_count, uint32_t slot) {
    return slot == 0u && alloc_count > 1u && indirection[1] == indirection[0];
}

KJB_KERNEL(256) k_ircache_clear_pool(uint32_t* pool, uint32_t* life, Rows kjb_rows) {
    const uint32_t idx = tid1d(); if (idx >= MAX_ENTRIES) return;
    pool[idx] = idx; life[idx] = IRCACHE_ENTRY_LIFE_RECYCLED;
}

KJB_DEV void ircache_scroll_cell(const Globals& g, const uint32_t* gm, uint32_t* gm2, uint32_t* entry_cell, float4* irradiance, uint32_t* life, uint32_t* pool, uint32_t* meta, uint32_t dst_cell_idx,
                                 bool parallel = false) {
    const uint32_t x = dst_cell_idx & 31u, y = (dst_cell_idx >> 5) & 31u, z = (dst_cell_idx >> 10) & 31u, cascade = dst_cell_idx >> 15;
    const int32_t* sb = g.fc.ircache_cascades[cascade].voxels_scrolled_this_frame;
    const uint32_t ox = x - uint32_t(sb[0]), oy = y - uint32_t(sb[1]), oz = z - uint32_t(sb[2]);
    if (!(ox < 32u && oy < 32u && oz < 32u)) {
        const uint32_t m0 = gm[dst_cell_idx * 2], m1 = gm[dst_cell_idx * 2 + 1];
// ... 72 lines not shown
KJB_KERNEL(256) k_ircache_age(uint32_t* meta, uint32_t* gm, uint32_t* entry_cell, uint32_t* life, uint32_t* pool, float4* spatial, float4* proposal, uint32_t* proposal_count,
                              float4* irradiance, uint32_t* occupancy, float4* entry_vertex, Rows kjb_rows) {
    if constexpr (SERIAL) KJB_SERIAL_1D(MAX_ENTRIES, ircache_age_entry(meta, gm, entry_cell, life, pool, spatial, proposal, proposal_count, irradiance, occupancy, i, entry_vertex));
    else { const uint32_t i = tid1d(); if (i < MAX_ENTRIES) ircache_age_entry(meta, gm, entry_cell, life, pool, spatial, proposal, proposal_count, irradiance, occupancy, i, entry_vertex); }
}

KJB_KERNEL(256) k_ircache_det_free(uint32_t* life, uint32_t* life_pending, uint32_t* free_scan, Rows kjb_rows) {
    const uint32_t e = tid1d(); if (e >= MAX_ENTRIES) return;
    uint32_t l = life[e];
    const uint32_t p = life_pending[e];
    if (p) {
        const uint32_t nl = IRCACHE_ENTRY_LIFE_RECYCLE - p;
        if (l < IRCACHE_ENTRY_LIFE_RECYCLE && nl < l) life[e] = l = nl;
        life_pending[e] = 0;
    }
    free_scan[e] = l == IRCACHE_ENTRY_LIFE_RECYCLED ? 1u : 0u;
}
KJB_KERNEL(256) k_ircache_det_pool(const uint32_t* free_scan, uint32_t* pool, uint32_t* meta, Rows kjb_rows) {
    const uint32_t e = tid1d(); if (e >= MAX_ENTRIES) return;
    const uint32_t base = MAX_ENTRIES - free_scan[MAX_ENTRIES - 1];
    if (e == 0) meta[IRCACHE_META_ALLOC_COUNT] = base;
    if (free_scan[e] != (e ? free_scan[e - 1] : 0u)) pool[base + free_scan[e] - 1] = e;
}
KJB_KERNEL(256) k_ircache_det_claims(const uint32_t* claim_rank, uint32_t* claim_bits, uint32_t* claim_scan, Rows kjb_rows) {
    const uint32_t w = tid1d(); if (w >= KJB_IRCACHE_GRID_CELLS / 32) return;
    uint32_t m = 0;
    for (uint32_t k = 0; k < 32; ++k) m |= (claim_rank[w * 32 + k] ? 1u : 0u) << k;
    claim_bits[w] = m; claim_scan[w] = kjb_popc(m);
}
KJB_KERNEL(256) k_ircache_det_assign(uint32_t* meta, uint32_t* gm, uint32_t* entry_cell, uint32_t* life, const uint32_t* pool, float4* entry_vertex, uint32_t* claim_rank, float4* claim_vertex,
                                     const uint32_t* free_scan, const uint32_t* claim_bits, const uint32_t* claim_scan, Rows kjb_rows) {
    const uint32_t cell = tid1d(); if (cell >= KJB_IRCACHE_GRID_CELLS) return;
    const uint32_t w = cell >> 5, k = cell & 31u, m = claim_bits[w];
    if (!((m >> k) & 1u)) return;
    const uint32_t n = (w ? claim_scan[w - 1] : 0u) + kjb_popc(m & ((1u << k) - 1u));
    const uint32_t free_count = free_scan[MAX_ENTRIES - 1];
    const uint32_t rank = IRCACHE_ENTRY_RANK_COUNT - claim_rank[cell];
    const float4 v = claim_vertex[cell];
    claim_rank[cell] = 0; claim_vertex[cell] = f4(0.0f);
    if (n >= free_count) { atom_and(&gm[cell * 2 + 1], ~(IRCACHE_ENTRY_META_OCCUPIED | IRCACHE_ENTRY_META_JUST_ALLOCATED)); return; }
    const uint32_t entry_idx = pool[MAX_ENTRIES - free_count + n];
    atom_max(&meta[IRCACHE_META_ENTRY_COUNT], entry_idx + 1);
    atom_add(&meta[IRCACHE_META_ALLOC_COUNT], 1u);
    life[entry_idx] = ircache_entry_life_for_rank(rank);
    entry_cell[entry_idx] = cell;
    gm[cell * 2 + 0] = entry_idx;
    entry_vertex[entry_idx] = v;
}
KJB_KERNEL(256) k_ircache_det_snapshot_aux(const uint32_t* meta, const float4* aux, float4* aux_prev, Rows kjb_rows) {
    const uint32_t i = tid1d(), e = i / 32u; if (e >= MAX_ENTRIES || e >= meta[IRCACHE_META_ENTRY_COUNT]) return;
    aux_prev[i] = aux[e * IRCACHE_AUX_STRIDE + i % 32u];
}

#define KJB_SCAN_CHUNKS 8
KJB_KERNEL(1024) k_inclusive_prefix_scan(uint32_t* d, uint32_t n, Rows kjb_rows) {
    __shared__ uint32_t warp_tot[KJB_SCAN_CHUNKS][32];
    const uint32_t t = threadIdx.x;
    const bool vec = (reinterpret_cast<uintptr_t>(d) & 15u) == 0;
    uint32_t v[KJB_SCAN_CHUNKS][8], s[KJB_SCAN_CHUNKS];
#pragma unroll
    for (uint32_t c = 0; c < KJB_SCAN_CHUNKS; ++c) {
        const uint32_t b = c * 8192u + t * 8u;
        if (vec && b + 8u <= n) {
            const uint4 lo = *reinterpret_cast<const uint4*>(d + b), hi = *reinterpret_cast<const uint4*>(d + b + 4);
            v[c][0] = lo.x; v[c][1] = lo.y; v[c][2] = lo.z; v[c][3] = lo.w; v[c][4] = hi.x; v[c][5] = hi.y; v[c][6] = hi.z; v[c][7] = hi.w;
        } else {
#pragma unroll
            for (uint32_t k = 0; k < 8u; ++k) v[c][k] = b + k < n ? d[b + k] : 0u;
        }
    }
#pragma unroll
    for (uint32_t c = 0; c < KJB_SCAN_CHUNKS; ++c) {
        uint32_t a = 0;
#pragma unroll
        for (uint32_t k = 0; k < 8u; ++k) { a += v[c][k]; v[c][k] = a; }
        s[c] = a;
    }
    uint32_t before[KJB_SCAN_CHUNKS];
#if !defined(KJB_EMU)
    const uint32_t lane = t & 31u, warp = t >> 5;
    uint32_t inc[KJB_SCAN_CHUNKS];
#pragma unroll
    for (uint32_t c = 0; c < KJB_SCAN_CHUNKS; ++c) {
        uint32_t a = s[c];
#pragma unroll
        for (uint32_t off = 1; off < 32u; off <<= 1) { const uint32_t u = __shfl_up_sync(0xffffffffu, a, off); if (lane >= off) a += u; }
        inc[c] = a;
        if (lane == 31u) warp_tot[c][warp] = a;
    }
    __syncthreads();
    if (warp < KJB_SCAN_CHUNKS) {
        uint32_t a = warp_tot[warp][lane];
#pragma unroll
        for (uint32_t off = 1; off < 32u; off <<= 1) { const uint32_t u = __shfl_up_sync(0xffffffffu, a, off); if (lane >= off) a += u; }
        warp_tot[warp][lane] = a;
    }
    __syncthreads();
    uint32_t carry = 0;
#pragma unroll
    for (uint32_t c = 0; c < KJB_SCAN_CHUNKS; ++c) {
        before[c] = carry + (warp ? warp_tot[c][warp - 1] : 0u) + (inc[c] - s[c]);
        carry += warp_tot[c][31];
    }
#else
    static thread_local uint32_t tot[KJB_SCAN_CHUNKS * 1024];
    (void)warp_tot;
    for (uint32_t c = 0; c < KJB_SCAN_CHUNKS; ++c) tot[c * 1024u + t] = s[c];
    __syncthreads();
    if (t == 0) { uint32_t a = 0; for (uint32_t i = 0; i < KJB_SCAN_CHUNKS * 1024u; ++i) { const uint32_t x = tot[i]; tot[i] = a; a += x; } }
    __syncthreads();
    for (uint32_t c = 0; c < KJB_SCAN_CHUNKS; ++c) before[c] = tot[c * 1024u + t];
    __syncthreads();
#endif
#pragma unroll
    for (uint32_t c = 0; c < KJB_SCAN_CHUNKS; ++c) {
        const uint32_t b = c * 8192u + t * 8u;
        if (vec && b + 8u <= n) {
            *reinterpret_cast<uint4*>(d + b) = make_uint4(v[c][0] + before[c], v[c][1] + before[c], v[c][2] + before[c], v[c][3] + before[c]);
            *reinterpret_cast<uint4*>(d + b + 4) = make_uint4(v[c][4] + before[c], v[c][5] + before[c], v[c][6] + before[c], v[c][7] + before[c]);
        } else {
#pragma unroll
            for (uint32_t k = 0; k < 8u; ++k) if (b + k < n) d[b + k] = v[c][k] + before[c];
        }
    }
}

KJB_KERNEL(256) k_ircache_compact(const uint32_t* meta, const uint32_t* life, const uint32_t* occupancy, uint32_t* indirection, Rows kjb_rows) {
    const uint32_t entry_idx = tid1d(); if (entry_idx >= MAX_ENTRIES) return;
    const uint32_t total_entry_count = meta[IRCACHE_META_ENTRY_COUNT];
    if (entry_idx < total_entry_count && is_ircache_entry_life_valid(life[entry_idx])) indirection[occupancy[entry_idx]] = entry_idx;
}

KJB_KERNEL(256) k_ircache_reset(const uint32_t* meta, const float4* irradiance, float4* aux, const uint32_t* indirection, Rows kjb_rows) {
    const uint32_t gid = tid1d(), dispatch_idx = gid / IRCACHE_AUX_STRIDE, i = gid % IRCACHE_AUX_STRIDE;
    const uint32_t alloc_count = meta[IRCACHE_META_TRACING_ALLOC_COUNT];
    if (dispatch_idx >= alloc_count || ircache_slot_is_stale_duplicate(indirection, alloc_count, dispatch_idx)) return;
    const uint32_t entry_idx = indirection[dispatch_idx];
    const float4 v = irradiance[entry_idx * IRCACHE_IRRADIANCE_STRIDE];
    if (v.x == 0.0f && v.y == 0.0f && v.z == 0.0f && v.w == 0.0f) aux[entry_idx * IRCACHE_AUX_STRIDE + i] = f4(0.0f);
}

KJB_KERNEL(128) k_ircache_trace_access(const __grid_constant__ Globals g, const float4* spatial, const uint32_t* life, const uint32_t* meta, float4* aux, const uint32_t* indirection, Rows kjb_rows) {
    const uint32_t dispatch_idx = tid1d();
    const uint32_t alloc_count = meta[IRCACHE_META_TRACING_ALLOC_COUNT];
    if (dispatch_idx >= alloc_count * IRCACHE_OCTA_DIMS2 || dispatch_idx >= MAX_ENTRIES * IRCACHE_OCTA_DIMS2) return;
    if (ircache_slot_is_stale_duplicate(indirection, alloc_count, dispatch_idx / IRCACHE_OCTA_DIMS2)) return;
    const uint32_t entry_idx = indirection[dispatch_idx / IRCACHE_OCTA_DIMS2], octa_idx = dispatch_idx % IRCACHE_OCTA_DIMS2;
    if (!is_ircache_entry_life_valid(life[entry_idx])) return;
    const IrcacheVertex entry = unpack_vertex(spatial[entry_idx]);
    const uint32_t output_idx = entry_idx * IRCACHE_AUX_STRIDE + octa_idx;
    const float4 ra = aux[output_idx];
    Reservoir r = Reservoir::from_raw(u2(kjb_f2u(ra.x), kjb_f2u(ra.y)));
    const IrcacheVertex prev_entry = unpack_vertex(aux[output_idx + IRCACHE_OCTA_DIMS2 * 2]);
    if (rt_is_shadowed(g, entry.position, prev_entry.position - entry.position, 0.001f, 0.999f)) {
        r.M *= 0.8f;
        const uint2 raw = r.as_raw();
        aux[output_idx] = f4(kjb_u2f(raw.x), kjb_u2f(raw.y), ra.z, ra.w);
    }
}

struct IrcacheTraceResult { float3 incident_radiance, direction, hit_pos; };
KJB_DEV IrcacheTraceResult ircache_trace(const Globals& g, const IrcacheBufs& b, const Img& sky_cube_tex, const IrcacheVertex& entry, SampleParams sample_params, uint32_t life) {
    uint32_t rng = sample_params.rng();
    Ray outgoing_ray; outgoing_ray.origin = entry.position; outgoing_ray.dir = sample_params.direction(); outgoing_ray.tmin = 0.0f; outgoing_ray.tmax = KJB_FLT_MAX;
    IrcacheTraceResult result; result.direction = outgoing_ray.dir; result.hit_pos = f3(0.0f);
    float3 irradiance_sum = f3(0.0f);
    RayCone cone; cone.width = 0; cone.spread_angle = 0.1f;
    const GbufferPathVertex primary_hit = gbuffer_raytrace(g, outgoing_ray, cone, 1, false);
    if (primary_hit.is_hit) {
        result.hit_pos = primary_hit.position;
        const float3 to_light_norm = sun_direction(g.fc);
        const bool is_shadowed = rt_is_shadowed(g, primary_hit.position, to_light_norm, 1e-4f, KJB_FLT_MAX);
        const GbufferData gbuffer = gbuffer_unpack(primary_hit.gbuffer_packed);
        const float3x3 tangent_to_world = build_orthonormal_basis(gbuffer.normal);
        const float3 wi = mul(to_light_norm, tangent_to_world);
        float3 wo = mul(-outgoing_ray.dir, tangent_to_world);
        if (wo.z < 0.0f) { wo.z *= -0.25f; wo = normalize(wo); }
        LayeredBrdf brdf = layered_brdf_from_gbuffer_ndotv(g, gbuffer, wo.z);
        brdf.specular_brdf.roughness = kjb_lerp(brdf.specular_brdf.roughness, 1.0f, 0.5f);
        const float3 brdf_value = layered_evaluate_directional_light(brdf, wo, wi);
        const float3 light_radiance = is_shadowed ? f3(0.0f) : f3(g.sun_color[0], g.sun_color[1], g.sun_color[2]);
        irradiance_sum += brdf_value * light_radiance * kjb_max(0.0f, wi.z);
        irradiance_sum += gbuffer.emissive;
        if (g.fc.triangle_light_count > 0) {
            const float light_selection_pmf = 1.0f / float(g.fc.triangle_light_count);
            const uint32_t light_idx = hash1_mut(rng) % g.fc.triangle_light_count;
            float2 urand; urand.x = rand01(rng); urand.y = rand01(rng);
            const kjb_triangle_light tl = g.lights[light_idx];
            const LightSample ls = sample_triangle_light(tl, urand);
            const float3 to_light_ws = ls.pos - primary_hit.position;
            const float dist_to_light2 = dot(to_light_ws, to_light_ws);
            const float3 to_light_norm_ws = to_light_ws * kjb_rsqrt(dist_to_light2);
            const float to_psa_metric = kjb_max(0.0f, dot(to_light_norm_ws, gbuffer.normal)) * kjb_max(0.0f, dot(to_light_norm_ws, -ls.normal)) / dist_to_light2;
            if (to_psa_metric > 0.0f) {
                const float3 wi2 = mul(to_light_norm_ws, tangent_to_world);
                const bool sh = rt_is_shadowed(g, primary_hit.position, to_light_norm_ws, 1e-3f, kjb_sqrt(dist_to_light2) - 2e-3f);
                irradiance_sum += sh ? f3(0.0f) : f3(tl.radiance[0], tl.radiance[1], tl.radiance[2]) * layered_evaluate(brdf, wo, wi2) / ls.pdf * to_psa_metric / light_selection_pmf;
            }
        }
        irradiance_sum += ircache_lookup<true>(g, b, entry.position, primary_hit.position, gbuffer.normal, 1 + ircache_entry_life_to_rank(life), rng) * gbuffer.albedo;
    } else {
        result.hit_pos = outgoing_ray.origin + outgoing_ray.dir * 1000.0f;
        irradiance_sum += xyz(sample_cube_rgba16f(sky_cube_tex, outgoing_ray.dir));
    }
    result.incident_radiance = irradiance_sum;
    return result;
}
KJB_DEV float self_lighting_limiter(float3 dir, float3 normal) { return kjb_lerp(0.5f, 1.0f, kjb_smoothstep(-0.1f, 0.0f, dot(dir, normal))); }

KJB_DEV void ircache_validate_sample(const Globals& g, const IrcacheBufs& b, const Img& sky_cube_tex, const uint32_t* indirection, uint32_t dispatch_idx) {
    const uint32_t alloc_count = b.meta[IRCACHE_META_TRACING_ALLOC_COUNT];
    if (dispatch_idx >= alloc_count * IRCACHE_VALIDATION_SAMPLES_PER_FRAME || dispatch_idx >= MAX_ENTRIES * IRCACHE_VALIDATION_SAMPLES_PER_FRAME) return;
    if (ircache_slot_is_stale_duplicate(indirection, alloc_count, dispatch_idx / IRCACHE_VALIDATION_SAMPLES_PER_FRAME)) return;
    const uint32_t entry_idx = indirection[dispatch_idx / IRCACHE_VALIDATION_SAMPLES_PER_FRAME], sample_idx = dispatch_idx % IRCACHE_VALIDATION_SAMPLES_PER_FRAME;
    const uint32_t life = b.life[entry_idx];
    const SampleParams sample_params = SampleParams::from_spf_entry_sample_frame(IRCACHE_VALIDATION_SAMPLES_PER_FRAME, entry_idx, sample_idx, g.fc.frame_index);
    const uint32_t output_idx = entry_idx * IRCACHE_AUX_STRIDE + sample_params.octa_idx();
    const float4 ra = b.aux[output_idx];
    Reservoir r = Reservoir::from_raw(u2(kjb_f2u(ra.x), kjb_f2u(ra.y)));
    if (r.M > 0) {
        const float ped = g.fc.pre_exposure_delta;
        float4 prev_value_and_count = b.aux[output_idx + IRCACHE_OCTA_DIMS2] * f4(ped, ped, ped, 1);
        const IrcacheVertex prev_entry = unpack_vertex(b.aux[output_idx + IRCACHE_OCTA_DIMS2 * 2]);
        const IrcacheTraceResult prev_traced = ircache_trace(g, b, sky_cube_tex, prev_entry, SampleParams::from_raw(r.payload), life);
        const float3 av = prev_traced.incident_radiance * self_lighting_limiter(prev_traced.direction, prev_entry.normal), bv = xyz(prev_value_and_count);
        const float3 dist3 = vabs(av - bv) / (av + bv);
        const float dist = kjb_max(dist3.x, kjb_max(dist3.y, dist3.z));
        const float invalidity = kjb_smoothstep(0.1f, 0.5f, dist);
        r.M = kjb_max(0.0f, kjb_min(r.M, kjb_exp2(kjb_log2(float(IRCACHE_RESTIR_M_CLAMP)) * (1.0f - invalidity))));
        prev_value_and_count = f4(av, prev_value_and_count.w);
        const uint2 raw = r.as_raw();
        b.aux[output_idx] = f4(kjb_u2f(raw.x), kjb_u2f(raw.y), ra.z, ra.w);
        b.aux[output_idx + IRCACHE_OCTA_DIMS2] = prev_value_and_count;
    }
}
template <bool SERIAL>
KJB_KERNEL(128) k_ircache_validate(const __grid_constant__ Globals g, IrcacheBufs b, Img sky_cube_tex, const uint32_t* indirection, Rows kjb_rows) {
    if constexpr (SERIAL) {
        const uint32_t n = b.meta[IRCACHE_META_TRACING_ALLOC_COUNT] * IRCACHE_VALIDATION_SAMPLES_PER_FRAME, n_max = MAX_ENTRIES * IRCACHE_VALIDATION_SAMPLES_PER_FRAME;
        KJB_SERIAL_1D(n < n_max ? n : n_max, ircache_validate_sample(g, b, sky_cube_tex, indirection, i));
    } else ircache_validate_sample(g, b, sky_cube_tex, indirection, tid1d());
}

KJB_DEV void ircache_trace_sample(const Globals& g, const IrcacheBufs& b, const Img& sky_cube_tex, const uint32_t* indirection, uint32_t dispatch_idx) {
    const uint32_t alloc_count = b.meta[IRCACHE_META_TRACING_ALLOC_COUNT];
    if (dispatch_idx >= alloc_count * IRCACHE_SAMPLES_PER_FRAME || dispatch_idx >= MAX_ENTRIES * IRCACHE_SAMPLES_PER_FRAME) return;
    if (ircache_slot_is_stale_duplicate(indirection, alloc_count, dispatch_idx / IRCACHE_SAMPLES_PER_FRAME)) return;
    const uint32_t entry_idx = indirection[dispatch_idx / IRCACHE_SAMPLES_PER_FRAME], sample_idx = dispatch_idx % IRCACHE_SAMPLES_PER_FRAME;
    const uint32_t life = b.life[entry_idx];
    const float4 packed_entry = b.spatial[entry_idx];
    const IrcacheVertex entry = unpack_vertex(packed_entry);
    uint32_t rng = hash1(hash1(entry_idx) + g.fc.frame_index);
    const SampleParams sample_params = SampleParams::from_spf_entry_sample_frame(IRCACHE_SAMPLES_PER_FRAME, entry_idx, sample_idx, g.fc.frame_index);
    const IrcacheTraceResult traced = ircache_trace(g, b, sky_cube_tex, entry, sample_params, life);
    const float3 new_value = traced.incident_radiance * self_lighting_limiter(traced.direction, entry.normal);
    const float new_lum = luminance(new_value);
    StreamState stream_state; Reservoir reservoir = Reservoir::create();
    reservoir.init_with_stream(new_lum, 1.0f, stream_state, sample_params.value);
    const uint32_t output_idx = entry_idx * IRCACHE_AUX_STRIDE + sample_params.octa_idx();
    const float ped = g.fc.pre_exposure_delta;
    const float4 prev_value_and_count = b.aux[output_idx + IRCACHE_OCTA_DIMS2] * f4(ped, ped, ped, 1);
    float3 val_sel = new_value; bool selected_new = true;
    const float4 ra = b.aux[output_idx];
    {
        Reservoir r = Reservoir::from_raw(u2(kjb_f2u(ra.x), kjb_f2u(ra.y)));
        if (r.M > 0) {
            r.M = kjb_min(r.M, 30.0f);
            if (reservoir.update_with_stream(r, luminance(xyz(prev_value_and_count)), 1.0f, stream_state, r.payload, rng)) { val_sel = xyz(prev_value_and_count); selected_new = false; }
        }
    }
    reservoir.finish_stream(stream_state);
    const uint2 raw = reservoir.as_raw();
    b.aux[output_idx] = f4(kjb_u2f(raw.x), kjb_u2f(raw.y), ra.z, ra.w);
    b.aux[output_idx + IRCACHE_OCTA_DIMS2] = f4(val_sel, reservoir.W);
    if (selected_new) b.aux[output_idx + IRCACHE_OCTA_DIMS2 * 2] = packed_entry;
}
template <bool SERIAL>
KJB_KERNEL(128) k_ircache_trace(const __grid_constant__ Globals g, IrcacheBufs b, Img sky_cube_tex, const uint32_t* indirection, Rows kjb_rows) {
    if constexpr (SERIAL) {
        const uint32_t n = b.meta[IRCACHE_META_TRACING_ALLOC_COUNT] * IRCACHE_SAMPLES_PER_FRAME, n_max = MAX_ENTRIES * IRCACHE_SAMPLES_PER_FRAME;
        KJB_SERIAL_1D(n < n_max ? n : n_max, ircache_trace_sample(g, b, sky_cube_tex, indirection, i));
    } else ircache_trace_sample(g, b, sky_cube_tex, indirection, tid1d());
}

KJB_KERNEL(256) k_ircache_sum(const __grid_constant__ Globals g, const uint32_t* meta, float4* irradiance, const float4* aux, const uint32_t* indirection, Rows kjb_rows) {
    const uint32_t dispatch_idx = tid1d();
    const uint32_t alloc_count = meta[IRCACHE_META_TRACING_ALLOC_COUNT];
    if (dispatch_idx >= alloc_count || dispatch_idx >= MAX_ENTRIES || ircache_slot_is_stale_duplicate(indirection, alloc_count, dispatch_idx)) return;
    const uint32_t entry_idx = indirection[dispatch_idx];
    float4 sh_rgb[3] = {f4(0.0f), f4(0.0f), f4(0.0f)};
    float valid_samples = 0;
    for (uint32_t octa_idx = 0; octa_idx < IRCACHE_OCTA_DIMS2; ++octa_idx) {
        const float4 ra = aux[entry_idx * IRCACHE_AUX_STRIDE + octa_idx];
        const Reservoir r = Reservoir::from_raw(u2(kjb_f2u(ra.x), kjb_f2u(ra.y)));
        const float3 dir = SampleParams::from_raw(r.payload).direction();
        const float4 contrib = aux[entry_idx * IRCACHE_AUX_STRIDE + IRCACHE_OCTA_DIMS2 + octa_idx];
        const float3 radiance = xyz(contrib) * contrib.w;
        const float4 sh = f4(0.282095f, dir.x * 0.488603f, dir.y * 0.488603f, dir.z * 0.488603f) * 4.0f;
        sh_rgb[0] += sh * radiance.x; sh_rgb[1] += sh * radiance.y; sh_rgb[2] += sh * radiance.z;
        valid_samples += contrib.w > 0 ? 1.0f : 0.0f;
    }
    const float sc = 1.0f / kjb_max(1.0f, valid_samples);
    const float ped = g.fc.pre_exposure_delta;
    for (uint32_t basis_i = 0; basis_i < IRCACHE_IRRADIANCE_STRIDE; ++basis_i) {
        const float4 new_value = sh_rgb[basis_i] * sc;
        float4 prev_value = irradiance[entry_idx * IRCACHE_IRRADIANCE_STRIDE + basis_i] * ped;
        const bool should_reset = !(prev_value.x != 0.0f || prev_value.y != 0.0f || prev_value.z != 0.0f || prev_value.w != 0.0f);
        if (should_reset) prev_value = new_value;
        irradiance[entry_idx * IRCACHE_IRRADIANCE_STRIDE + basis_i] = vlerp(prev_value, new_value, 0.25f);
    }
}

KJB_KERNEL(256) k_ircache_export_requests(IrcacheBufs b, uint32_t* block, uint32_t max_records, Rows kjb_rows) {
    const uint32_t e = tid1d();
    if (e >= b.meta[IRCACHE_META_ENTRY_COUNT] || e >= MAX_ENTRIES) return;
    const uint32_t life = b.life[e];
    if (!is_ircache_entry_life_valid(life) || ircache_entry_life_to_rank(life) > 1u) return;
    const uint32_t slot = atom_add(&block[0], 1u);
    if (slot >= max_records) return;
    uint32_t* rec = block + 4 + slot * 8u;
    float4 v = b.reposition_proposal[e];
    if (!(kjb_f2u(v.x) | kjb_f2u(v.y) | kjb_f2u(v.z) | kjb_f2u(v.w))) v = b.spatial[e];
    rec[0] = b.entry_cell[e]; rec[1] = life; rec[2] = b.reposition_count[e]; rec[3] = 0u;
    rec[4] = kjb_f2u(v.x); rec[5] = kjb_f2u(v.y); rec[6] = kjb_f2u(v.z); rec[7] = kjb_f2u(v.w);
}
KJB_KERNEL(256) k_ircache_merge_requests(IrcacheBufs b, const uint32_t* block, uint32_t max_records, uint32_t seed, Rows kjb_rows) {
    const uint32_t i = tid1d();
    const uint32_t n = block[0] < max_records ? block[0] : max_records;
    if (i >= n) return;
    const uint32_t* rec = block + 4 + i * 8u;
    const uint32_t cell_idx = rec[0], life_r = rec[1], count_r = rec[2];
    if (cell_idx >= KJB_IRCACHE_GRID_CELLS || !is_ircache_entry_life_valid(life_r)) return;
    const float4 vote = f4(kjb_u2f(rec[4]), kjb_u2f(rec[5]), kjb_u2f(rec[6]), kjb_u2f(rec[7]));
    if (b.det && (b.grid_meta[cell_idx * 2 + 1] & (IRCACHE_ENTRY_META_OCCUPIED | IRCACHE_ENTRY_META_JUST_ALLOCATED)) != IRCACHE_ENTRY_META_OCCUPIED) {
        atom_or(&b.grid_meta[cell_idx * 2 + 1], IRCACHE_ENTRY_META_OCCUPIED | IRCACHE_ENTRY_META_JUST_ALLOCATED);
        atom_max(&b.claim_rank[cell_idx], IRCACHE_ENTRY_RANK_COUNT - ircache_entry_life_to_rank(life_r));
        vertex_vote(&b.claim_vertex[cell_idx], vote);
        return;
    }
    bool fresh = false;
    if ((b.grid_meta[cell_idx * 2 + 1] & IRCACHE_ENTRY_META_OCCUPIED) == 0) {
        const uint32_t prev = atom_or(&b.grid_meta[cell_idx * 2 + 1], IRCACHE_ENTRY_META_OCCUPIED | IRCACHE_ENTRY_META_JUST_ALLOCATED);
        if ((prev & IRCACHE_ENTRY_META_OCCUPIED) == 0) {
            const uint32_t alloc_idx = atom_add(&b.meta[IRCACHE_META_ALLOC_COUNT], 1u);
            if (alloc_idx >= 1024u * 64u) {
                atom_add(&b.meta[IRCACHE_META_ALLOC_COUNT], uint32_t(-1));
                atom_and(&b.grid_meta[cell_idx * 2 + 1], ~(IRCACHE_ENTRY_META_OCCUPIED | IRCACHE_ENTRY_META_JUST_ALLOCATED));
                return;
            }
// ... 180 lines not shown
```

kajiya_b200/csrc/kjb_trace.cuh:

```cuda
#pragma once
#include "kjb_device.cuh"
#include "kjb_bvh.h"

namespace kjb {

struct Ray { float3 origin, dir; float tmin, tmax; };
struct HitInfo { bool hit; float t, u, v; uint32_t gid; };

KJB_DEV void write_padded_slot(BvhNode& nd, int k, const float* b) {
    float lo[3], hi[3];
    for (int a = 0; a < 3; ++a) {
        const float pad = (b[3 + a] - b[a]) * 1e-5f + 1e-6f + 1e-6f * kjb_max(kjb_abs(b[a]), kjb_abs(b[3 + a]));
        lo[a] = b[a] - pad; hi[a] = b[3 + a] + pad;
    }
    float* nxy = k == 0 ? nd.n0 : nd.n1;
    nxy[0] = lo[0]; nxy[1] = hi[0]; nxy[2] = lo[1]; nxy[3] = hi[1];
    nd.n2[k * 2 + 0] = lo[2]; nd.n2[k * 2 + 1] = hi[2];
}

KJB_DEV float4 ldg4(const float* p) {
#if defined(__CUDA_ARCH__)
    return __ldg(reinterpret_cast<const float4*>(p));
#else
    return f4(p[0], p[1], p[2], p[3]);
#endif
}

template <bool ANY_HIT>
KJB_DEV bool intersect_leaf(const BvhTri* tris, uint32_t first, uint32_t count, const Ray& r, bool cull_back, HitInfo& best) {
    for (uint32_t i = 0; i < count; ++i) {
        const float* tp = reinterpret_cast<const float*>(tris + first + i);
        const float4 a = ldg4(tp), b = ldg4(tp + 4), c = ldg4(tp + 8);
        const float3 v0 = f3(a.x, a.y, a.z), e1 = f3(b.x, b.y, b.z), e2 = f3(c.x, c.y, c.z);
        const float3 p = cross(r.dir, e2);
        const float det = dot(e1, p);
        if (det == 0.0f) continue;
        if (cull_back && det < 0.0f) continue;
        const float inv = 1.0f / det;
        const float3 tv = r.origin - v0;
        const float u = dot(tv, p) * inv;
        if (u < 0.0f || u > 1.0f) continue;
        const float3 q = cross(tv, e1);
        const float v = dot(r.dir, q) * inv;
        if (v < 0.0f || u + v > 1.0f) continue;
        const float t = dot(e2, q) * inv;
        if (!(t > r.tmin && t < r.tmax)) continue;
        if (ANY_HIT) return true;
        const uint32_t gid = kjb_f2u(a.w);
        if (!best.hit || t < best.t || (t == best.t && gid < best.gid)) { best.hit = true; best.t = t; best.u = u; best.v = v; best.gid = gid; }
    }
    return false;
}

#define KJB_SLAB_MIN kjb_min
#define KJB_SLAB_MAX kjb_max

#define KJB_SLAB_SLACK_K 16384.0f
KJB_DEV float slab_near(float t) { return kjb_fma(-KJB_SLAB_SLACK_K * 0x1p-24f, kjb_abs(t), t); }
KJB_DEV float slab_far(float t) { return kjb_fma(KJB_SLAB_SLACK_K * 0x1p-24f, kjb_abs(t), t); }
template <bool ANY_HIT>
KJB_DEV HitInfo trace(const SceneView& sc, const Ray& r, bool cull_back) {
    HitInfo best; best.hit = false; best.t = r.tmax; best.u = 0; best.v = 0; best.gid = 0xffffffffu;
    if (!(r.dir.x == r.dir.x && r.dir.y == r.dir.y && r.dir.z == r.dir.z && r.origin.x == r.origin.x && r.origin.y == r.origin.y && r.origin.z == r.origin.z
          && r.tmin == r.tmin && r.tmax == r.tmax)) return best;
    const float3 inv_dir = f3(1.0f / r.dir.x, 1.0f / r.dir.y, 1.0f / r.dir.z);
    int stack[64]; int sp = 0;
    int cur = sc.root;
    const int DONE = 0x7fffffff;
    for (;;) {
        while (cur >= 0 && cur != DONE) {
            const float* np = reinterpret_cast<const float*>(sc.nodes + cur);
            const float4 n0 = ldg4(np), n1 = ldg4(np + 4), n2 = ldg4(np + 8);
            const int2 ch = *reinterpret_cast<const int2*>(np + 12);
            const float c0lox = (n0.x - r.origin.x) * inv_dir.x, c0hix = (n0.y - r.origin.x) * inv_dir.x;
            const float c0loy = (n0.z - r.origin.y) * inv_dir.y, c0hiy = (n0.w - r.origin.y) * inv_dir.y;
            const float c0loz = (n2.x - r.origin.z) * inv_dir.z, c0hiz = (n2.y - r.origin.z) * inv_dir.z;
            const float c1lox = (n1.x - r.origin.x) * inv_dir.x, c1hix = (n1.y - r.origin.x) * inv_dir.x;
            const float c1loy = (n1.z - r.origin.y) * inv_dir.y, c1hiy = (n1.w - r.origin.y) * inv_dir.y;
            const float c1loz = (n2.z - r.origin.z) * inv_dir.z, c1hiz = (n2.w - r.origin.z) * inv_dir.z;
            const float tmax_cur = ANY_HIT ? r.tmax : best.t;
            const float t0n = slab_near(KJB_SLAB_MAX(KJB_SLAB_MAX(KJB_SLAB_MIN(c0lox, c0hix), KJB_SLAB_MIN(c0loy, c0hiy)), KJB_SLAB_MAX(KJB_SLAB_MIN(c0loz, c0hiz), r.tmin)));
            const float t0f = slab_far(KJB_SLAB_MIN(KJB_SLAB_MIN(KJB_SLAB_MAX(c0lox, c0hix), KJB_SLAB_MAX(c0loy, c0hiy)), KJB_SLAB_MIN(KJB_SLAB_MAX(c0loz, c0hiz), tmax_cur)));
            const float t1n = slab_near(KJB_SLAB_MAX(KJB_SLAB_MAX(KJB_SLAB_MIN(c1lox, c1hix), KJB_SLAB_MIN(c1loy, c1hiy)), KJB_SLAB_MAX(KJB_SLAB_MIN(c1loz, c1hiz), r.tmin)));
            const float t1f = slab_far(KJB_SLAB_MIN(KJB_SLAB_MIN(KJB_SLAB_MAX(c1lox, c1hix), KJB_SLAB_MAX(c1loy, c1hiy)), KJB_SLAB_MIN(KJB_SLAB_MAX(c1loz, c1hiz), tmax_cur)));
            const bool h0 = t0n <= t0f, h1 = t1n <= t1f;
            if (h0 && h1) {
                const bool near0 = t0n <= t1n;
                stack[sp++] = near0 ? ch.y : ch.x;
                cur = near0 ? ch.x : ch.y;
            } else if (h0) cur = ch.x;
            else if (h1) cur = ch.y;
            else cur = sp ? stack[--sp] : DONE;
        }
        if (cur == DONE) break;
        {
            const uint32_t enc = uint32_t(~cur);
            if (intersect_leaf<ANY_HIT>(sc.tris, enc >> 3, (enc & 7u) + 1u, r, cull_back, best)) { best.hit = true; return best; }
        }
        cur = sp ? stack[--sp] : DONE;
    }
    return best;
}

KJB_DEV void count_ray(const SceneView& sc, int which) {
#if defined(__CUDA_ARCH__)
    const unsigned m = __activemask();
    if ((threadIdx.x + threadIdx.y * blockDim.x) % 32 == __ffs(m) - 1) atomicAdd(sc.ray_counters + which, (unsigned long long)__popc(m));
#else
    __atomic_fetch_add(sc.ray_counters + which, 1ull, __ATOMIC_RELAXED);
#endif
}

KJB_DEV float srgb_eotf(float a) { return .04045f < a ? kjb_pow((a + .055f) / 1.055f, 2.4f) : a / 12.92f; }
KJB_DEV float4 tex_texel(const SceneView& sc, uint4 d, int mip, int x, int y) {
    const int w = int(d.y >> mip) > 1 ? int(d.y >> mip) : 1, h = int(d.z >> mip) > 1 ? int(d.z >> mip) : 1;
    x = ((x % w) + w) % w; y = ((y % h) + h) % h;
    size_t off = d.x;
    for (int m = 0; m < mip; ++m) { const size_t mw = (d.y >> m) > 1 ? (d.y >> m) : 1, mh = (d.z >> m) > 1 ? (d.z >> m) : 1; off += mw * mh * 4; }
    const uint8_t* p = sc.tex_data + off + (size_t(y) * w + x) * 4;
    float4 c = f4(float(p[0]) / 255.0f, float(p[1]) / 255.0f, float(p[2]) / 255.0f, float(p[3]) / 255.0f);
    if (d.w >> 16) { c.x = srgb_eotf(c.x); c.y = srgb_eotf(c.y); c.z = srgb_eotf(c.z); }
    return c;
}
KJB_DEV float4 tex_bilinear_repeat(const SceneView& sc, uint4 d, int mip, float2 uv) {
    const int w = int(d.y >> mip) > 1 ? int(d.y >> mip) : 1, h = int(d.z >> mip) > 1 ? int(d.z >> mip) : 1;
    const float fx = uv.x * float(w) - 0.5f, fy = uv.y * float(h) - 0.5f;
    const float x0f = kjb_floor(fx), y0f = kjb_floor(fy); const float tx = fx - x0f, ty = fy - y0f;
    const int x0 = kjb_cvt_i32(x0f), y0 = kjb_cvt_i32(y0f);
    const float4 a = tex_texel(sc, d, mip, x0, y0), b = tex_texel(sc, d, mip, x0 + 1, y0), c = tex_texel(sc, d, mip, x0, y0 + 1), e = tex_texel(sc, d, mip, x0 + 1, y0 + 1);
    const float4 top = a + (b - a) * tx, bot = c + (e - c) * tx;
    return top + (bot - top) * ty;
}
KJB_DEV float4 tex_sample_level(const SceneView& sc, uint32_t tex, float2 uv, float lod) {
    if (tex >= sc.tex_count) return f4(1.0f);
    const uint4 d = sc.tex_desc[tex];
    const int mips = int(d.w & 0xffffu);
    if (mips == 1 && d.y == 1u && d.z == 1u) return tex_texel(sc, d, 0, 0, 0);
    const float maxl = float(mips - 1);
    if (!(lod > 0.0f)) lod = 0.0f;
    if (lod > maxl) lod = maxl;
    const int l0 = kjb_cvt_i32(kjb_floor(lod)); const float f = lod - float(l0);
    const float4 a = tex_bilinear_repeat(sc, d, l0, uv);
    if (f == 0.0f || l0 + 1 >= mips) return a;
    const float4 b = tex_bilinear_repeat(sc, d, l0 + 1, uv);
    return a + (b - a) * f;
}
KJB_DEV float texture_lod(const SceneView& sc, uint32_t tex, float triangle_constant, float3 ray_direction, float3 surf_normal, float cone_width) {
    float2 wh = f2(1.0f);
    if (tex < sc.tex_count) { const uint4 d = sc.tex_desc[tex]; wh = f2(float(d.y), float(d.z)); }
    float lambda = triangle_constant;
    lambda += kjb_log2(kjb_abs(cone_width));
    lambda += 0.5f * kjb_log2(wh.x * wh.y);
    lambda -= kjb_log2(kjb_abs(dot(normalize(ray_direction), surf_normal)));
    return lambda;
}

KJB_DEV uint32_t vb_u32(const SceneView& sc, uint32_t off) { return *reinterpret_cast<const uint32_t*>(sc.vertices + off); }
KJB_DEV float vb_f32(const SceneView& sc, uint32_t off) { return *reinterpret_cast<const float*>(sc.vertices + off); }
KJB_DEV float3 unpack_unit_direction_11_10_11(uint32_t pck) {
    return f3(float(pck & ((1u << 11u) - 1u)) * (2.0f / float((1u << 11u) - 1u)) - 1.0f,
              float((pck >> 11u) & ((1u << 10u) - 1u)) * (2.0f / float((1u << 10u) - 1u)) - 1.0f,
              float((pck >> 21u)) * (2.0f / float((1u << 11u) - 1u)) - 1.0f);
}
KJB_DEV float2 transform_material_uv(const float* t, float2 uv, uint32_t map_idx) {
    const uint32_t xo = map_idx * 6;
    return f2(t[xo + 0] * uv.x + t[xo + 1] * uv.y, t[xo + 2] * uv.x + t[xo + 3] * uv.y) + f2(t[xo + 4], t[xo + 5]);
}

KJB_DEV uint4 rchit_gbuffer(const Globals& g, const Ray& ray, const HitInfo& hit, RayCone ray_cone, uint32_t path_length, float3* geometric_normal_ws_out = nullptr) {
    const SceneView& sc = g.scene;
    const TriInfo ti = sc.tri_info[hit.gid];
    const kjb_instance& inst = sc.instances[ti.instance];
    const kjb_gpu_mesh mesh = sc.meshes[inst.mesh_index];
    const float* o2w = inst.transform;
    const float3 hit_point = ray.origin + ray.dir * hit.t;
    const float hit_dist = length(hit_point - ray.origin);
    const float3 bary = f3(1.0f - hit.u - hit.v, hit.u, hit.v);

    uint32_t ind[3];
    for (int k = 0; k < 3; ++k) ind[k] = vb_u32(sc, mesh.index_offset + (ti.prim * 3 + k) * 4);
    float3 vp[3], vn[3];
    for (int k = 0; k < 3; ++k) {
        const float4 v = *reinterpret_cast<const float4*>(sc.vertices + mesh.vertex_core_offset + ind[k] * 16);
        vp[k] = f3(v.x, v.y, v.z); vn[k] = unpack_unit_direction_11_10_11(kjb_f2u(v.w));
    }
    float3 normal = vn[0] * bary.x + vn[1] * bary.y + vn[2] * bary.z;
    const float3 surf_normal_os = normalize(cross(vp[1] - vp[0], vp[2] - vp[0]));
    const float3 surf_normal_ws = normalize(xform_dir(o2w, surf_normal_os));
    if (g.fc.render_override_flags & KJB_OVERRIDE_FORCE_FACE_NORMALS) normal = surf_normal_os;

    float4 v_color = f4(1.0f);
    if (mesh.vertex_aux_offset != 0) {
        float4 vc[3];
        for (int k = 0; k < 3; ++k) vc[k] = *reinterpret_cast<const float4*>(sc.vertices + mesh.vertex_aux_offset + ind[k] * 16);
        v_color = vc[0] * bary.x + vc[1] * bary.y + vc[2] * bary.z;
    }
    float2 uvs[3];
    for (int k = 0; k < 3; ++k) uvs[k] = *reinterpret_cast<const float2*>(sc.vertices + mesh.vertex_uv_offset + ind[k] * 8);
    const float2 uv = uvs[0] * bary.x + uvs[1] * bary.y + uvs[2] * bary.z;

    const uint32_t material_id = vb_u32(sc, mesh.vertex_mat_offset + ind[0] * 4);
    const kjb_mesh_material& material = *reinterpret_cast<const kjb_mesh_material*>(sc.vertices + mesh.mat_data_offset + material_id * (uint32_t)sizeof(kjb_mesh_material));

#ifndef KJB_LOD_SKIP
#define KJB_LOD_SKIP 1
#endif
    auto flat = [&](uint32_t tex) { if (!KJB_LOD_SKIP) return false; if (tex >= sc.tex_count) return true; const uint4 d = sc.tex_desc[tex]; return (d.w & 0xffffu) == 1u && d.y == 1u && d.z == 1u; };
    const bool any_filtered = !flat(material.maps[2]) || !flat(material.maps[1]) || !flat(material.maps[3]);
    float cone_width = 0.0f, lod_triangle_constant = 0.0f;
    if (any_filtered) {
        cone_width = ray_cone.width + ray_cone.spread_angle * hit_dist;
        const float3 p0 = xform_point(o2w, vp[0]), p1 = xform_point(o2w, vp[1]), p2 = xform_point(o2w, vp[2]);
        const float twice_uv_area = kjb_abs((uvs[1].x - uvs[0].x) * (uvs[2].y - uvs[0].y) - (uvs[2].x - uvs[0].x) * (uvs[1].y - uvs[0].y));
        const float twice_triangle_area = length(cross(p1 - p0, p2 - p0));
        lod_triangle_constant = 0.5f * kjb_log2(twice_uv_area / twice_triangle_area);
    }
    auto sample_map = [&](uint32_t tex, uint32_t uv_slot) {
        if (flat(tex)) return tex_sample_level(sc, tex, f2(0.0f), 0.0f);
        return tex_sample_level(sc, tex, transform_material_uv(material.map_transforms, uv, uv_slot), texture_lod(sc, tex, lod_triangle_constant, ray.dir, surf_normal_ws, cone_width));
    };

    const float3 albedo = xyz(sample_map(material.maps[2], 0))
        * f3(material.base_color_mult[0], material.base_color_mult[1], material.base_color_mult[2]) * xyz(v_color);

    const float4 metalness_roughness = sample_map(material.maps[1], 2);
    const float perceptual_roughness = material.roughness_mult * metalness_roughness.x;
    float roughness = kjb_clamp(perceptual_roughness * perceptual_roughness, 1e-4f, 1.0f);
    float metalness = metalness_roughness.y * material.metalness_factor;
    if (g.fc.render_override_flags & KJB_OVERRIDE_NO_METAL) metalness = 0;
    const float rs = g.fc.render_override_material_roughness_scale;
    if (rs <= 1) roughness *= rs; else roughness = square(kjb_lerp(kjb_sqrt(roughness), 1.0f, 1.0f - 1.0f / rs));

    float3 emissive = f3(0.0f);
    if (0 == path_length || 0 == (material.flags & 1u)) {
        emissive = f3(1.0f) * xyz(sample_map(material.maps[3], 3))
            * f3(material.emissive[0], material.emissive[1], material.emissive[2]) * inst.emissive_multiplier * g.fc.pre_exposure;
    }
    GbufferData gb;
    gb.albedo = albedo;
    gb.normal = normalize(xform_dir(o2w, normal));
    gb.roughness = roughness; gb.metalness = metalness; gb.emissive = emissive;
    if (dot(ray.dir, gb.normal) > 0) gb.normal = gb.normal * -1.0f;
    if (geometric_normal_ws_out) *geometric_normal_ws_out = surf_normal_ws;
    return gbuffer_pack(gb);
}

struct GbufferPathVertex { bool is_hit; uint4 gbuffer_packed; float3 position; float ray_t; };
KJB_DEV GbufferPathVertex gbuffer_raytrace(const Globals& g, const Ray& ray, RayCone cone, uint32_t path_length, bool cull_back_faces) {
    count_ray(g.scene, 0);
    const HitInfo h = trace<false>(g.scene, ray, cull_back_faces);
    GbufferPathVertex r;
    if (h.hit) {
        r.is_hit = true; r.position = ray.origin + ray.dir * h.t; r.gbuffer_packed = rchit_gbuffer(g, ray, h, cone, path_length); r.ray_t = h.t;
    } else { r.is_hit = false; r.ray_t = KJB_FLT_MAX; r.gbuffer_packed = u4(0, 0, 0, 0); r.position = f3(0.0f); }
    return r;
}
KJB_DEV bool rt_is_shadowed(const Globals& g, float3 origin, float3 dir, float tmin, float tmax) {
    count_ray(g.scene, 1);
    Ray r; r.origin = origin; r.dir = dir; r.tmin = tmin; r.tmax = tmax;
    return trace<true>(g.scene, r, false).hit;
}

}
```

kajiya_b200/world.py:

```python
import ctypes as C
import numpy as np
from ._abi import Image, WorldDesc, WorldFrame, MeshDesc, MeshMaterial, TextureDesc, FMT_NUMPY, KjbError


def quat_from_rotation_x(angle):
    return (float(np.sin(angle / 2)), 0.0, 0.0, float(np.cos(angle / 2)))


class World:
    def __init__(self, lib, width, height, device=0, spatial_reuse_pass_count=2, enable_ircache=False, enable_rtr=False, enable_taa=False,
                 upscale=None, tile=None, use_raytraced_reservoir_visibility=False, enable_ssao=False, enable_lighting=False, hard_sun=False):
        self.lib = lib
        self.d = lib.dll
        self.ctx = C.c_void_p()
        if self.d.kjb_create(device, C.byref(self.ctx)):
            raise KjbError("kjb_create failed: " + (self.d.kjb_last_error(None) or b"").decode())
        tile_rank, tile_count = tile if tile else (0, 0)
        desc = WorldDesc(width, height, (upscale or (0, 0))[0], (upscale or (0, 0))[1], spatial_reuse_pass_count, int(use_raytraced_reservoir_visibility),
                         int(enable_ircache), int(enable_rtr), int(enable_taa), 0, 0, tile_rank, tile_count, int(enable_ssao), int(enable_lighting), int(hard_sun))
        self.w = C.c_void_p()
        if tile_count > 1 and enable_lighting:
            raise KjbError("tile-sharded frames do not include the lit composite (enable_lighting): DESIGN.md §7")
        self._check(self.d.kjb_world_create(self.ctx, C.byref(desc), C.byref(self.w)))
        self.width, self.height = width, height
# ... 36 lines not shown
        mats = (MeshMaterial * len(mesh["materials"]))()
        maps = []
        texel_keep = []
        for i, m in enumerate(mesh["materials"]):
            mm = mats[i]
            mm.base_color_mult[:] = m.get("base_color", [1, 1, 1, 1])
            mm.roughness_mult = m.get("roughness", 1.0); mm.metalness_factor = m.get("metallic", 1.0)
            mm.emissive[:] = m.get("emissive", [0, 0, 0]); mm.flags = 0
            for k in range(4):
                mm.map_transforms[k * 6:(k + 1) * 6] = [1, 0, 0, 1, 0, 0]
            placeholders = [(127, 127, 255, 255), (255, 255, 127, 255), (255, 255, 255, 255), (255, 255, 255, 255)]
            for k, key in enumerate(("normal_map", "spec_map", "albedo_map", "emissive_map")):
                tex = m.get(key)
                if tex is None:
                    texels = np.array([placeholders[k]], np.uint8); w = h = mips = 1; srgb = 0
                else:
                    texels, w, h, mips, srgb = tex
                texels = np.ascontiguousarray(texels, np.uint8); texel_keep.append(texels)
                maps.append(TextureDesc(texels.ctypes.data, w, h, mips, srgb))
                mm.maps[k] = len(maps) - 1
        maps_arr = (TextureDesc * len(maps))(*maps)
        md = MeshDesc(pos.ctypes.data, nrm.ctypes.data, uvs.ctypes.data if uvs is not None else None, col.ctypes.data if col is not None else None,
                      mid.ctypes.data, idx.ctypes.data, len(pos), len(idx), mats, len(mats), maps_arr, len(maps), int(use_lights))
        h = C.c_uint32()
        self._check(self.d.kjb_world_add_mesh(self.w, C.byref(md), C.byref(h)))
        return h.value

    def add_mesh_desc(self, desc, use_lights=False):
        desc.use_lights = int(use_lights)
        h = C.c_uint32()
        self._check(self.d.kjb_world_add_mesh(self.w, C.byref(desc), C.byref(h)))
        return h.value

    def add_instance(self, mesh, transform3x4):
        t = (C.c_float * 12)(*np.asarray(transform3x4, np.float32).reshape(12))
        h = C.c_uint32()
        self._check(self.d.kjb_world_add_instance(self.w, mesh, C.byref(t), C.byref(h)))
        return h.value

    def set_instance_transform(self, handle, transform):
        t = (C.c_float * 12)(*np.asarray(transform, np.float32).reshape(-1)[:12])
        self._check(self.d.kjb_world_set_instance_transform(self.w, handle, C.byref(t)))

    def set_sun_color_multiplier(self, rgb):
        self._check(self.d.kjb_world_set_sun_color_multiplier(self.w, C.byref((C.c_float * 3)(*rgb))))

    def set_sky_ambient(self, rgb):
        self._check(self.d.kjb_world_set_sky_ambient(self.w, C.byref((C.c_float * 3)(*rgb))))

    def set_render_overrides(self, flags=0, material_roughness_scale=1.0):
        self._check(self.d.kjb_world_set_render_overrides(self.w, int(flags), float(material_roughness_scale)))

    def reset_reference_accumulation(self):
        self._check(self.d.kjb_world_reset_reference_accumulation(self.w))

    def set_debug_shading_mode(self, mode):
        self._check(self.d.kjb_world_set_debug_shading_mode(self.w, int(mode)))

    def set_sun_size_multiplier(self, m):
        self._check(self.d.kjb_world_set_sun_size_multiplier(self.w, float(m)))

    def remove_instance(self, handle):
        self._check(self.d.kjb_world_remove_instance(self.w, handle))

    def set_instance_emissive_multiplier(self, handle, value):
        self._check(self.d.kjb_world_set_instance_emissive_multiplier(self.w, handle, float(value)))

    def set_blue_noise(self, rgba8):
        a = np.ascontiguousarray(rgba8, np.uint8); assert a.size == 256 * 256 * 4
        self._check(self.d.kjb_world_set_blue_noise(self.w, a.ctypes.data))

    def _frame(self, camera_position, camera_rotation, sun_direction, vfov=52.0, host_inputs=None, host_result=None, capture_slot=0, replay_slot=0, streaming=False):
        f = WorldFrame()
        f.camera_position[:] = camera_position; f.camera_rotation[:] = camera_rotation
        f.vertical_fov_deg = vfov; f.near_plane = 0.01; f.sun_direction[:] = sun_direction; f.delta_time_seconds = 1.0 / 60.0
        if host_inputs is not None:
            f.host_gbuffer, f.host_depth, f.host_geometric_normal, f.host_velocity = host_inputs
        if host_result is not None:
            f.host_result = host_result
        f.capture_slot, f.replay_slot = capture_slot, replay_slot
        f.streaming = int(streaming)
        return f

    def render_frame(self, camera_position, camera_rotation, sun_direction, **kw):
        f = self._frame(camera_position, camera_rotation, sun_direction, **kw)
        self._check(self.d.kjb_world_render_frame(self.w, C.byref(f)))

    def render_reference(self, camera_position, camera_rotation, sun_direction, indirect_only=False, **kw):
        f = self._frame(camera_position, camera_rotation, sun_direction, **kw)
        self._check(self.d.kjb_world_render_reference(self.w, C.byref(f), int(indirect_only)))

    def wait(self):
        self._check(self.d.kjb_world_wait(self.w))

    def sync(self):
        self._check(self.d.kjb_sync(self.ctx))

    def set_profiling(self, on):
        self.d.kjb_world_set_profiling(self.w, int(on))

    def pass_timings(self):
        out = {}
        for line in self.d.kjb_world_pass_timings(self.w).decode().split("\n"):
            if line:
                label, calls, ms = line.split("\t"); out[label] = (int(calls), float(ms))
        return out

    def timer_record(self, slot):
        self._check(self.d.kjb_timer_record(self.ctx, slot))

    def timer_elapsed_ms(self, a, b):
        ms = C.c_float()
        self._check(self.d.kjb_timer_elapsed_ms(self.ctx, a, b, C.byref(ms)))
        return ms.value

    def stop_after(self, label):
        self.d.kjb_world_set_stop_after(self.w, (label or "").encode())

    @property
    def frame_index(self):
        return self.d.kjb_world_frame_index(self.w)

    def stats(self):
        s = (C.c_uint64 * 4)()
        self.d.kjb_world_last_frame_stats(self.w, C.byref(s))
        return dict(launches=s[0], closest_rays=s[1], any_hit_rays=s[2], passes=s[3])

    def set_cuda_graph(self, on):
        self._check(self.d.kjb_world_set_cuda_graph(self.w, int(on)))

    def set_async_compute(self, on):
        self._check(self.d.kjb_world_set_async_compute(self.w, int(on)))

    def graph_stats(self):
        s = (C.c_uint64 * 2)()
        self._check(self.d.kjb_graph_stats(self.ctx, C.byref(s)))
        return dict(launches=s[0], instantiations=s[1])

    def tlas_stats(self):
        s = (C.c_uint64 * 2)()
        self._check(self.d.kjb_tlas_stats(self.ctx, C.byref(s)))
        return dict(rebuilds=s[0], refits=s[1])

    def tlas_download(self):
        if not self.lib.has_tlas_download:
            raise KjbError(f"{self.lib.backend} does not expose its acceleration structure")
        counts, root = (C.c_uint32 * 3)(), C.c_int32()
        self._check(self.d.kjb_tlas_download(self.ctx, C.byref(counts), C.byref(root), None, None, None, None))
        nodes, tris = np.zeros((counts[0], 16), np.uint32), np.zeros((counts[1], 12), np.uint32)
        info, parent = np.zeros((counts[2], 2), np.uint32), np.zeros(counts[0], np.int32)
        self._check(self.d.kjb_tlas_download(self.ctx, C.byref(counts), C.byref(root), nodes.ctypes.data, tris.ctypes.data, info.ctypes.data, parent.ctypes.data))
        return dict(nodes=nodes, tris=tris, tri_info=info, parent=parent, root=int(root.value))

    def trace_rays(self, rays, any_hit=False, cull_back=False, brute_force=False):
        if not self.lib.has_tlas_trace:
            raise KjbError(f"{self.lib.backend} does not expose its acceleration structure")
        r = np.ascontiguousarray(rays, np.float32).reshape(-1, 8)
        out = np.zeros((len(r), 4), np.uint32)
        flags = (1 if any_hit else 0) | (2 if cull_back else 0) | (4 if brute_force else 0)
        self._check(self.d.kjb_tlas_trace(self.ctx, r.ctypes.data, len(r), flags, out.ctypes.data))
        return out

    def image_names(self):
        return [n for n in self.d.kjb_world_image_names(self.w).decode().split("\n") if n]

    def image_handle(self, name):
        img = Image()
        if self.d.kjb_world_get_image(self.w, name.encode(), C.byref(img)):
            raise KeyError(name)
        return img

    def image(self, name):
        img = self.image_handle(name)
        dt, comps = FMT_NUMPY[img.format]
        out = np.empty((img.layers * img.height, img.width, comps), dt)
        self._check(self.d.kjb_image_download(self.ctx, C.byref(img), out.ctypes.data))
        self.sync()
        return out
```

Measured before the change: 548.5 million.

## Collapse binary BVH into 4-wide BVH and traverse it for ircache rays

Builds a 4-wide BVH by collapsing every other level of the binary BVH on device, using a depth-parity flag, a prefix scan and a fill kernel. The wide tree is refreshed on refit. A new SoA-layout wide traversal tests four child boxes per node and sorts hits by entry distance. It is used for ircache trace and shadow rays and as the default for the trace API. The aim is to halve traversal steps and memory round-trips per ray, at the cost of extra build and refit kernels, more memory, and a larger per-thread stack.

After: 551.6 million (median of 6 runs). About the same (+0.6%).

```diff
diff --git a/include/kjb_tlas.h b/include/kjb_tlas.h
--- a/include/kjb_tlas.h
+++ b/include/kjb_tlas.h
@@ -6,9 +6,12 @@
 #endif
 int kjb_tlas_download(kjb_context *ctx, uint32_t out_counts[3], int32_t *out_root, void *nodes, void *tris, void *tri_info, int32_t *parent);
 
+int kjb_tlas_download_wide(kjb_context *ctx, uint32_t *out_count, int32_t *out_root, void *nodes);
+
 #define KJB_TLAS_TRACE_ANY_HIT 1u
 #define KJB_TLAS_TRACE_CULL_BACK 2u
 #define KJB_TLAS_TRACE_BRUTE_FORCE 4u
+#define KJB_TLAS_TRACE_BINARY 8u
 int kjb_tlas_trace(kjb_context *ctx, const float *rays, uint32_t n, uint32_t flags, float *out);
 #ifdef __cplusplus
 }
diff --git a/kajiya_b200/_abi.py b/kajiya_b200/_abi.py
--- a/kajiya_b200/_abi.py
+++ b/kajiya_b200/_abi.py
@@ -131,6 +131,10 @@
         if self.has_tlas_download:
             d.kjb_tlas_download.restype = C.c_int
             d.kjb_tlas_download.argtypes = [P, C.POINTER(C.c_uint32 * 3), C.POINTER(C.c_int32), P, P, P, P]
+        self.has_tlas_download_wide = hasattr(d, "kjb_tlas_download_wide")
+        if self.has_tlas_download_wide:
+            d.kjb_tlas_download_wide.restype = C.c_int
+            d.kjb_tlas_download_wide.argtypes = [P, C.POINTER(C.c_uint32), C.POINTER(C.c_int32), P]
         self.has_tlas_trace = hasattr(d, "kjb_tlas_trace")
         if self.has_tlas_trace:
             d.kjb_tlas_trace.restype = C.c_int
diff --git a/kajiya_b200/csrc/kjb_api.cu b/kajiya_b200/csrc/kjb_api.cu
--- a/kajiya_b200/csrc/kjb_api.cu
+++ b/kajiya_b200/csrc/kjb_api.cu
@@ -62,6 +62,58 @@
     }
 }
 
+KJB_KERNEL(256) k_wide_flags(const int32_t* parent, const uint32_t* node_count, uint32_t bound, uint32_t* flags, Rows kjb_rows) {
+    const uint32_t i = blockIdx.x * blockDim.x + threadIdx.x;
+    if (i >= bound) return;
+    if (i >= *node_count) { flags[i] = 0; return; }
+    uint32_t depth = 0;
+    for (int32_t p = parent[i]; p >= 0; p = parent[p >> 1]) ++depth;
+    flags[i] = (depth & 1u) ? 0u : 1u;
+}
+KJB_KERNEL(256) k_wide_map(const uint32_t* scan, const uint32_t* tiles, const uint32_t* node_count, int32_t* map, uint32_t* wide_count, Rows kjb_rows) {
+    const uint32_t i = blockIdx.x * blockDim.x + threadIdx.x, n = *node_count;
+    if (i == 0) *wide_count = n ? bvhb::scan_incl(scan, tiles, n - 1) : 0u;
+    if (i >= n) return;
+    const uint32_t before = bvhb::scan_excl(scan, tiles, i);
+    map[i] = bvhb::scan_incl(scan, tiles, i) > before ? int32_t(before) : -1;
+}
+KJB_KERNEL(256) k_wide_fill(const BvhNode* nodes, const int32_t* map, const uint32_t* node_count, BvhWideNode* wide, Rows kjb_rows) {
+    const uint32_t i = blockIdx.x * blockDim.x + threadIdx.x;
+    if (i >= *node_count) return;
+    const int32_t w = map[i];
+    if (w < 0) return;
+    BvhWideNode o; memset(&o, 0, sizeof(o));
+    int m = 0;
+    auto put = [&](const BvhNode& nd, int k) {
+        const float* xy = k ? nd.n1 : nd.n0;
+        o.lox[m] = xy[0]; o.hix[m] = xy[1]; o.loy[m] = xy[2]; o.hiy[m] = xy[3]; o.loz[m] = nd.n2[2 * k]; o.hiz[m] = nd.n2[2 * k + 1];
+        o.child[m] = nd.child[k] >= 0 ? map[nd.child[k]] : nd.child[k];
+        ++m;
+    };
+    const BvhNode nd = nodes[i];
+    for (int k = 0; k < 2; ++k) {
+        if (nd.child[k] >= 0) { const BvhNode ch = nodes[nd.child[k]]; put(ch, 0); put(ch, 1); }
+        else put(nd, k);
+    }
+    for (; m < 4; ++m) o.child[m] = WIDE_EMPTY;
+    wide[w] = o;
+}
+static void collapse_wide(kjb_context* c, bool topology) {
+    const uint32_t bound = c->node_count;
+    if (!bound) return;
+    const kjb::Rows kjb__rows = {0, 1};
+    const dim3 grid((bound + 255) / 256), b256(256);
+    if (topology) {
+        bvhb::View v; bvhb::carve(c->bvh_tri_cap, (uint8_t*)c->d_bvh_scratch, &v);
+        const uint32_t tiles = (bound + bvhb::TILE - 1) / bvhb::TILE;
+        KJB_LAUNCH(c, k_wide_flags, KJB_DIMS(grid, b256), (const int32_t*)c->d_node_parent, (const uint32_t*)c->d_node_count, bound, v.scan);
+        KJB_LAUNCH_SYNC(c, bvhb::k_bvhb_scan_tiles, KJB_DIMS(dim3(tiles), dim3(1024)), v.scan, bound, v.tiles, (const uint32_t*)nullptr);
+        KJB_LAUNCH_SYNC(c, bvhb::k_bvhb_scan_tile_totals, KJB_DIMS(dim3(1), dim3(1024)), v.tiles, tiles, (const uint32_t*)nullptr);
+        KJB_LAUNCH(c, k_wide_map, KJB_DIMS(grid, b256), (const uint32_t*)v.scan, (const uint32_t*)v.tiles, (const uint32_t*)c->d_node_count, c->d_wide_map, c->d_wide_count);
+    }
+    KJB_LAUNCH(c, k_wide_fill, KJB_DIMS(grid, b256), (const BvhNode*)c->d_nodes, (const int32_t*)c->d_wide_map, (const uint32_t*)c->d_node_count, c->d_wide);
+}
+
 extern "C" {
 
 int kjb_abi_version(void) { return KJB_ABI_VERSION; }
@@ -103,6 +155,7 @@
     dev_sync(c);
     dev_free(c->d_vertices); dev_free(c->d_meshes); dev_free(c->d_instances); dev_free(c->d_nodes); dev_free(c->d_tris); dev_free(c->d_tri_info);
     dev_free(c->d_node_parent); dev_free(c->d_refit_count); dev_free(c->d_slot_box); dev_free(c->d_tri_box); dev_free(c->d_bvh_scratch); dev_free(c->d_inst_prefix);
+    dev_free(c->d_wide); dev_free(c->d_wide_map);
     dev_free(c->d_tex_data); dev_free(c->d_tex_desc); dev_free(c->d_lights); dev_free(c->d_ray_counters); dev_free(c->d_prev_instances); dev_free(c->d_resolve_offsets);
     for (auto& kv : c->ircache_scratch) { const auto& s = kv.second; dev_free(s.claim_rank); dev_free(s.claim_vertex); dev_free(s.life_pending); dev_free(s.scan); dev_free(s.claim_bits); dev_free(s.aux_prev); dev_free(s.entry_vertex); }
 #if !defined(KJB_EMU)
@@ -267,13 +320,15 @@
     if (grow_tris) {
         const uint32_t cap = std::max(std::max(tris, 1u), c->bvh_tri_cap + c->bvh_tri_cap / 2);
         dev_free(c->d_nodes); dev_free(c->d_tris); dev_free(c->d_tri_info); dev_free(c->d_node_parent); dev_free(c->d_refit_count); dev_free(c->d_slot_box);
-        dev_free(c->d_tri_box); dev_free(c->d_bvh_scratch);
+        dev_free(c->d_tri_box); dev_free(c->d_bvh_scratch); dev_free(c->d_wide); dev_free(c->d_wide_map);
         c->d_nodes = (BvhNode*)dev_alloc(size_t(cap) * sizeof(BvhNode)); c->d_tris = (BvhTri*)dev_alloc(size_t(cap) * sizeof(BvhTri));
+        c->d_wide = (BvhWideNode*)dev_alloc(size_t(cap) * sizeof(BvhWideNode)); c->d_wide_map = (int32_t*)dev_alloc(size_t(cap + 1) * 4);
+        c->d_wide_count = c->d_wide_map ? (uint32_t*)(c->d_wide_map + cap) : nullptr;
         c->d_tri_info = (TriInfo*)dev_alloc(size_t(cap + 1) * sizeof(TriInfo)); c->d_node_parent = (int32_t*)dev_alloc(size_t(cap) * 4);
         c->d_refit_count = (uint32_t*)dev_alloc(size_t(cap) * 4); c->d_slot_box = (float*)dev_alloc(size_t(cap) * 12 * sizeof(float));
         c->d_tri_box = (float*)dev_alloc(size_t(cap) * 6 * sizeof(float)); c->d_bvh_scratch = dev_alloc(bvh_build_scratch_bytes(cap));
         c->bvh_tri_cap = cap;
-        if (!c->d_nodes || !c->d_tris || !c->d_tri_info || !c->d_node_parent || !c->d_refit_count || !c->d_slot_box || !c->d_tri_box || !c->d_bvh_scratch) {
+        if (!c->d_nodes || !c->d_tris || !c->d_tri_info || !c->d_node_parent || !c->d_refit_count || !c->d_slot_box || !c->d_tri_box || !c->d_bvh_scratch || !c->d_wide || !c->d_wide_map) {
             c->bvh_tri_cap = 0; return c->fail("kjb_rebuild_tlas: out of device memory");
         }
         c->d_node_count = bvh_build_node_count(c);
@@ -296,6 +351,7 @@
             const kjb::Rows kjb__rows = {0, 1};
             KJB_LAUNCH(c, k_refit_tris, KJB_DIMS(dim3((c->slot_count + 255) / 256), dim3(256)), c->g.scene, c->d_tris, c->d_tri_box, c->slot_count);
             KJB_LAUNCH(c, k_refit_nodes, KJB_DIMS(dim3((c->node_count + 255) / 256), dim3(256)), c->d_nodes, (const int32_t*)c->d_node_parent, c->d_refit_count, c->d_slot_box, (const float*)c->d_tri_box, (const uint32_t*)c->d_node_count);
+            collapse_wide(c, false);
             c->tlas_refits++;
             KJB_PASS_EPILOGUE(c, "rebuild tlas (refit)");
         }
@@ -318,7 +374,7 @@
     if ((n && dev_h2d(c, c->d_instances, stage, inst_bytes)) || dev_h2d(c, c->d_inst_prefix, prefix, size_t(n + 1) * 4)) return c->fail("kjb_rebuild_tlas: instance upload failed");
     c->tlas_rebuilds++;
     c->h_instances.assign(inst, inst + n);
-    c->g.scene.nodes = c->d_nodes; c->g.scene.tris = c->d_tris; c->g.scene.tri_info = c->d_tri_info; c->g.scene.instances = c->d_instances;
+    c->g.scene.nodes = c->d_nodes; c->g.scene.wide = c->d_wide; c->g.scene.tris = c->d_tris; c->g.scene.tri_info = c->d_tri_info; c->g.scene.instances = c->d_instances;
     c->g.scene.tri_count = ntri;
     c->g.scene.root = ntri == 0 ? ~int32_t(0) : (ntri <= 4 ? ~int32_t(ntri - 1) : 0);
     c->slot_count = ntri ? ntri : 1;
@@ -329,6 +385,7 @@
         KJB_PASS_EPILOGUE(c, "rebuild tlas");
     }
     if (bvh_build_on_device(c, n, ntri)) return 1;
+    collapse_wide(c, true);
     const kjb::Rows kjb__rows = {0, 1};
     KJB_LAUNCH(c, k_refit_tris, KJB_DIMS(dim3((ntri + 255) / 256), dim3(256)), c->g.scene, c->d_tris, c->d_tri_box, ntri);
     KJB_PASS_EPILOGUE(c, "rebuild tlas");
@@ -350,6 +407,18 @@
     const char* e = dev_check(c); if (e) return c->fail(std::string("kjb_tlas_download: ") + e);
     return 0;
 }
+int kjb_tlas_download_wide(kjb_context* c, uint32_t* out_count, int32_t* out_root, void* nodes) {
+    if (dev_sync(c)) return c->fail("kjb_tlas_download_wide: sync failed");
+    uint32_t n = 0;
+    if (c->tlas_valid && c->node_count) dev_d2h(c, &n, c->d_wide_count, 4);
+    if (dev_sync(c)) return c->fail("kjb_tlas_download_wide: sync failed");
+    *out_count = n;
+    if (out_root) *out_root = c->g.scene.root;
+    if (nodes && n) dev_d2h(c, nodes, c->d_wide, size_t(n) * sizeof(BvhWideNode));
+    if (dev_sync(c)) return c->fail("kjb_tlas_download_wide: sync failed");
+    const char* e = dev_check(c); if (e) return c->fail(std::string("kjb_tlas_download_wide: ") + e);
+    return 0;
+}
 
 }
 KJB_KERNEL(128) k_tlas_trace(SceneView sc, const float* rays, uint32_t n, uint32_t flags, uint32_t slots, uint32_t* out, Rows kjb_rows) {
@@ -362,8 +431,10 @@
     if (flags & KJB_TLAS_TRACE_BRUTE_FORCE) {
         if (any) h.hit = intersect_leaf<true>(sc.tris, 0, slots, r, cull, h);
         else intersect_leaf<false>(sc.tris, 0, slots, r, cull, h);
+    } else if (flags & KJB_TLAS_TRACE_BINARY) {
+        h = any ? trace_binary<true>(sc, r, cull) : trace_binary<false>(sc, r, cull);
     } else {
-        h = any ? trace<true>(sc, r, cull) : trace<false>(sc, r, cull);
+        h = any ? trace_wide<true>(sc, r, cull) : trace_wide<false>(sc, r, cull);
     }
     uint32_t* o = out + size_t(i) * 4;
     if (!h.hit) { o[0] = 0; o[1] = 0; o[2] = 0; o[3] = 0xffffffffu; }
@@ -374,7 +445,7 @@
 
 int kjb_tlas_trace(kjb_context* c, const float* rays, uint32_t n, uint32_t flags, float* out) {
     if (!c->tlas_valid) return c->fail("kjb_tlas_trace: no acceleration structure (render a frame or call kjb_rebuild_tlas first)");
-    if (flags & ~(KJB_TLAS_TRACE_ANY_HIT | KJB_TLAS_TRACE_CULL_BACK | KJB_TLAS_TRACE_BRUTE_FORCE)) return c->fail("kjb_tlas_trace: unknown flags");
+    if (flags & ~(KJB_TLAS_TRACE_ANY_HIT | KJB_TLAS_TRACE_CULL_BACK | KJB_TLAS_TRACE_BRUTE_FORCE | KJB_TLAS_TRACE_BINARY)) return c->fail("kjb_tlas_trace: unknown flags");
     if (n == 0) return 0;
     if (dev_sync(c)) return c->fail("kjb_tlas_trace: sync failed");
     float* d_rays = (float*)dev_alloc(size_t(n) * 8 * sizeof(float));
diff --git a/kajiya_b200/csrc/kjb_bvh.h b/kajiya_b200/csrc/kjb_bvh.h
--- a/kajiya_b200/csrc/kjb_bvh.h
+++ b/kajiya_b200/csrc/kjb_bvh.h
@@ -4,7 +4,10 @@
 namespace kjb {
 
 struct BvhNode { float n0[4], n1[4], n2[4]; int32_t child[4]; };
+struct BvhWideNode { float lox[4], hix[4], loy[4], hiy[4], loz[4], hiz[4]; int32_t child[4]; uint32_t spare[4]; };
 struct BvhTri { float v0[3]; uint32_t gid; float e1[3]; uint32_t pad0; float e2[3]; uint32_t pad1; };
 struct TriInfo { uint32_t instance, prim; };
 
+enum : int32_t { WIDE_EMPTY = 0x7fffffff };
+
 }
diff --git a/kajiya_b200/csrc/kjb_context.h b/kajiya_b200/csrc/kjb_context.h
--- a/kajiya_b200/csrc/kjb_context.h
+++ b/kajiya_b200/csrc/kjb_context.h
@@ -29,6 +29,7 @@
     kjb::BvhNode* d_nodes = nullptr; kjb::BvhTri* d_tris = nullptr; kjb::TriInfo* d_tri_info = nullptr;
     int32_t* d_node_parent = nullptr; uint32_t* d_refit_count = nullptr; float* d_slot_box = nullptr; float* d_tri_box = nullptr; uint32_t node_count = 0, slot_count = 0;
     uint64_t tlas_refits = 0, tlas_rebuilds = 0;
+    kjb::BvhWideNode* d_wide = nullptr; int32_t* d_wide_map = nullptr; uint32_t* d_wide_count = nullptr;
     uint32_t bvh_tri_cap = 0, bvh_inst_cap = 0; void* d_bvh_scratch = nullptr; uint32_t* d_inst_prefix = nullptr; uint32_t* d_node_count = nullptr;
     uint64_t staging_seq = 0;
     uint8_t* d_tex_data = nullptr; uint4* d_tex_desc = nullptr; uint32_t tex_count = 0;
diff --git a/kajiya_b200/csrc/kjb_device.cuh b/kajiya_b200/csrc/kjb_device.cuh
--- a/kajiya_b200/csrc/kjb_device.cuh
+++ b/kajiya_b200/csrc/kjb_device.cuh
@@ -371,10 +371,11 @@
 struct Rows { int y0, y1; };
 
 struct BvhNode;
+struct BvhWideNode;
 struct BvhTri;
 struct TriInfo;
 struct SceneView {
-    const BvhNode* nodes; const BvhTri* tris; const TriInfo* tri_info;
+    const BvhNode* nodes; const BvhWideNode* wide; const BvhTri* tris; const TriInfo* tri_info;
     const uint8_t* vertices; const kjb_gpu_mesh* meshes; const kjb_instance* instances;
     const uint8_t* tex_data; const uint4* tex_desc;
     uint32_t tex_count, tri_count;
diff --git a/kajiya_b200/csrc/kjb_passes_ircache.cu b/kajiya_b200/csrc/kjb_passes_ircache.cu
--- a/kajiya_b200/csrc/kjb_passes_ircache.cu
+++ b/kajiya_b200/csrc/kjb_passes_ircache.cu
@@ -248,7 +248,7 @@
     const float4 ra = aux[output_idx];
     Reservoir r = Reservoir::from_raw(u2(kjb_f2u(ra.x), kjb_f2u(ra.y)));
     const IrcacheVertex prev_entry = unpack_vertex(aux[output_idx + IRCACHE_OCTA_DIMS2 * 2]);
-    if (rt_is_shadowed(g, entry.position, prev_entry.position - entry.position, 0.001f, 0.999f)) {
+    if (rt_is_shadowed<Walk::wide>(g, entry.position, prev_entry.position - entry.position, 0.001f, 0.999f)) {
         r.M *= 0.8f;
         const uint2 raw = r.as_raw();
         aux[output_idx] = f4(kjb_u2f(raw.x), kjb_u2f(raw.y), ra.z, ra.w);
@@ -262,11 +262,11 @@
     IrcacheTraceResult result; result.direction = outgoing_ray.dir; result.hit_pos = f3(0.0f);
     float3 irradiance_sum = f3(0.0f);
     RayCone cone; cone.width = 0; cone.spread_angle = 0.1f;
-    const GbufferPathVertex primary_hit = gbuffer_raytrace(g, outgoing_ray, cone, 1, false);
+    const GbufferPathVertex primary_hit = gbuffer_raytrace<Walk::wide>(g, outgoing_ray, cone, 1, false);
     if (primary_hit.is_hit) {
         result.hit_pos = primary_hit.position;
         const float3 to_light_norm = sun_direction(g.fc);
-        const bool is_shadowed = rt_is_shadowed(g, primary_hit.position, to_light_norm, 1e-4f, KJB_FLT_MAX);
+        const bool is_shadowed = rt_is_shadowed<Walk::wide>(g, primary_hit.position, to_light_norm, 1e-4f, KJB_FLT_MAX);
         const GbufferData gbuffer = gbuffer_unpack(primary_hit.gbuffer_packed);
         const float3x3 tangent_to_world = build_orthonormal_basis(gbuffer.normal);
         const float3 wi = mul(to_light_norm, tangent_to_world);
@@ -290,7 +290,7 @@
             const float to_psa_metric = kjb_max(0.0f, dot(to_light_norm_ws, gbuffer.normal)) * kjb_max(0.0f, dot(to_light_norm_ws, -ls.normal)) / dist_to_light2;
             if (to_psa_metric > 0.0f) {
                 const float3 wi2 = mul(to_light_norm_ws, tangent_to_world);
-                const bool sh = rt_is_shadowed(g, primary_hit.position, to_light_norm_ws, 1e-3f, kjb_sqrt(dist_to_light2) - 2e-3f);
+                const bool sh = rt_is_shadowed<Walk::wide>(g, primary_hit.position, to_light_norm_ws, 1e-3f, kjb_sqrt(dist_to_light2) - 2e-3f);
                 irradiance_sum += sh ? f3(0.0f) : f3(tl.radiance[0], tl.radiance[1], tl.radiance[2]) * layered_evaluate(brdf, wo, wi2) / ls.pdf * to_psa_metric / light_selection_pmf;
             }
         }
diff --git a/kajiya_b200/csrc/kjb_trace.cuh b/kajiya_b200/csrc/kjb_trace.cuh
--- a/kajiya_b200/csrc/kjb_trace.cuh
+++ b/kajiya_b200/csrc/kjb_trace.cuh
@@ -59,7 +59,7 @@
 KJB_DEV float slab_near(float t) { return kjb_fma(-KJB_SLAB_SLACK_K * 0x1p-24f, kjb_abs(t), t); }
 KJB_DEV float slab_far(float t) { return kjb_fma(KJB_SLAB_SLACK_K * 0x1p-24f, kjb_abs(t), t); }
 template <bool ANY_HIT>
-KJB_DEV HitInfo trace(const SceneView& sc, const Ray& r, bool cull_back) {
+KJB_DEV HitInfo trace_binary(const SceneView& sc, const Ray& r, bool cull_back) {
     HitInfo best; best.hit = false; best.t = r.tmax; best.u = 0; best.v = 0; best.gid = 0xffffffffu;
     if (!(r.dir.x == r.dir.x && r.dir.y == r.dir.y && r.dir.z == r.dir.z && r.origin.x == r.origin.x && r.origin.y == r.origin.y && r.origin.z == r.origin.z
           && r.tmin == r.tmin && r.tmax == r.tmax)) return best;
@@ -102,6 +102,75 @@
     return best;
 }
 
+#define KJB_WIDE_STACK 99
+KJB_DEV bool wide_slab(const Ray& r, const float3 inv_dir, float tmax_cur, float nx, float fx, float ny, float fy, float nz, float fz, float& tn) {
+    const float cnx = (nx - r.origin.x) * inv_dir.x, cfx = (fx - r.origin.x) * inv_dir.x;
+    const float cny = (ny - r.origin.y) * inv_dir.y, cfy = (fy - r.origin.y) * inv_dir.y;
+    const float cnz = (nz - r.origin.z) * inv_dir.z, cfz = (fz - r.origin.z) * inv_dir.z;
+    tn = slab_near(KJB_SLAB_MAX(KJB_SLAB_MAX(cnx, cny), KJB_SLAB_MAX(cnz, r.tmin)));
+    const float tf = slab_far(KJB_SLAB_MIN(KJB_SLAB_MIN(cfx, cfy), KJB_SLAB_MIN(cfz, tmax_cur)));
+    return tn <= tf;
+}
+KJB_DEV void wide_cswap(float& ka, int& ca, float& kb, int& cb) {
+    const bool s = kb < ka;
+    const float k = s ? kb : ka; kb = s ? ka : kb; ka = k;
+    const int c = s ? cb : ca; cb = s ? ca : cb; ca = c;
+}
+template <bool ANY_HIT>
+KJB_DEV HitInfo trace_wide(const SceneView& sc, const Ray& r, bool cull_back) {
+    HitInfo best; best.hit = false; best.t = r.tmax; best.u = 0; best.v = 0; best.gid = 0xffffffffu;
+    if (!(r.dir.x == r.dir.x && r.dir.y == r.dir.y && r.dir.z == r.dir.z && r.origin.x == r.origin.x && r.origin.y == r.origin.y && r.origin.z == r.origin.z
+          && r.tmin == r.tmin && r.tmax == r.tmax)) return best;
+    const float3 inv_dir = f3(1.0f / r.dir.x, 1.0f / r.dir.y, 1.0f / r.dir.z);
+    const int ox = inv_dir.x < 0.0f ? 4 : 0, oy = inv_dir.y < 0.0f ? 12 : 8, oz = inv_dir.z < 0.0f ? 20 : 16;
+    int stack[KJB_WIDE_STACK]; int sp = 0;
+    int cur = sc.root;
+    const int DONE = 0x7fffffff;
+    for (;;) {
+        while (cur >= 0 && cur != DONE) {
+            const float* np = reinterpret_cast<const float*>(sc.wide + cur);
+            const float4 nx = ldg4(np + ox), fx = ldg4(np + (4 - ox)), ny = ldg4(np + oy), fy = ldg4(np + (20 - oy)), nz = ldg4(np + oz), fz = ldg4(np + (36 - oz));
+            const float4 chf = ldg4(np + 24);
+            int c0 = int(kjb_f2u(chf.x)), c1 = int(kjb_f2u(chf.y)), c2 = int(kjb_f2u(chf.z)), c3 = int(kjb_f2u(chf.w));
+            const float tmax_cur = ANY_HIT ? r.tmax : best.t;
+            const float INF = kjb_u2f(0x7f800000u);
+            float k0, k1, k2, k3;
+            const bool h0 = wide_slab(r, inv_dir, tmax_cur, nx.x, fx.x, ny.x, fy.x, nz.x, fz.x, k0) && c0 != WIDE_EMPTY;
+            const bool h1 = wide_slab(r, inv_dir, tmax_cur, nx.y, fx.y, ny.y, fy.y, nz.y, fz.y, k1) && c1 != WIDE_EMPTY;
+            const bool h2 = wide_slab(r, inv_dir, tmax_cur, nx.z, fx.z, ny.z, fy.z, nz.z, fz.z, k2) && c2 != WIDE_EMPTY;
+            const bool h3 = wide_slab(r, inv_dir, tmax_cur, nx.w, fx.w, ny.w, fy.w, nz.w, fz.w, k3) && c3 != WIDE_EMPTY;
+            if (ANY_HIT) {
+                if (h3) stack[sp++] = c3;
+                if (h2) stack[sp++] = c2;
+                if (h1) stack[sp++] = c1;
+                cur = h0 ? c0 : (sp ? stack[--sp] : DONE);
+                continue;
+            }
+            const int n = int(h0) + int(h1) + int(h2) + int(h3);
+            k0 = h0 ? k0 : INF; k1 = h1 ? k1 : INF; k2 = h2 ? k2 : INF; k3 = h3 ? k3 : INF;
+            wide_cswap(k0, c0, k1, c1); wide_cswap(k2, c2, k3, c3); wide_cswap(k0, c0, k2, c2); wide_cswap(k1, c1, k3, c3); wide_cswap(k1, c1, k2, c2);
+            if (n > 3) stack[sp++] = c3;
+            if (n > 2) stack[sp++] = c2;
+            if (n > 1) stack[sp++] = c1;
+            cur = n ? c0 : (sp ? stack[--sp] : DONE);
+        }
+        if (cur == DONE) break;
+        {
+            const uint32_t enc = uint32_t(~cur);
+            if (intersect_leaf<ANY_HIT>(sc.tris, enc >> 3, (enc & 7u) + 1u, r, cull_back, best)) { best.hit = true; return best; }
+        }
+        cur = sp ? stack[--sp] : DONE;
+    }
+    return best;
+}
+
+enum class Walk { binary, wide };
+template <bool ANY_HIT, Walk W = Walk::binary>
+KJB_DEV HitInfo trace(const SceneView& sc, const Ray& r, bool cull_back) {
+    if constexpr (W == Walk::wide) return trace_wide<ANY_HIT>(sc, r, cull_back);
+    else return trace_binary<ANY_HIT>(sc, r, cull_back);
+}
+
 KJB_DEV void count_ray(const SceneView& sc, int which) {
 #if defined(__CUDA_ARCH__)
     const unsigned m = __activemask();
@@ -246,19 +315,21 @@
 }
 
 struct GbufferPathVertex { bool is_hit; uint4 gbuffer_packed; float3 position; float ray_t; };
+template <Walk W = Walk::binary>
 KJB_DEV GbufferPathVertex gbuffer_raytrace(const Globals& g, const Ray& ray, RayCone cone, uint32_t path_length, bool cull_back_faces) {
     count_ray(g.scene, 0);
-    const HitInfo h = trace<false>(g.scene, ray, cull_back_faces);
+    const HitInfo h = trace<false, W>(g.scene, ray, cull_back_faces);
     GbufferPathVertex r;
     if (h.hit) {
         r.is_hit = true; r.position = ray.origin + ray.dir * h.t; r.gbuffer_packed = rchit_gbuffer(g, ray, h, cone, path_length); r.ray_t = h.t;
     } else { r.is_hit = false; r.ray_t = KJB_FLT_MAX; r.gbuffer_packed = u4(0, 0, 0, 0); r.position = f3(0.0f); }
     return r;
 }
+template <Walk W = Walk::binary>
 KJB_DEV bool rt_is_shadowed(const Globals& g, float3 origin, float3 dir, float tmin, float tmax) {
     count_ray(g.scene, 1);
     Ray r; r.origin = origin; r.dir = dir; r.tmin = tmin; r.tmax = tmax;
-    return trace<true>(g.scene, r, false).hit;
-}
-
-}
+    return trace<true, W>(g.scene, r, false).hit;
+}
+
+}
diff --git a/kajiya_b200/world.py b/kajiya_b200/world.py
--- a/kajiya_b200/world.py
+++ b/kajiya_b200/world.py
@@ -212,12 +212,21 @@
         self._check(self.d.kjb_tlas_download(self.ctx, C.byref(counts), C.byref(root), nodes.ctypes.data, tris.ctypes.data, info.ctypes.data, parent.ctypes.data))
         return dict(nodes=nodes, tris=tris, tri_info=info, parent=parent, root=int(root.value))
 
-    def trace_rays(self, rays, any_hit=False, cull_back=False, brute_force=False):
+    def tlas_download_wide(self):
+        if not self.lib.has_tlas_download_wide:
+            raise KjbError(f"{self.lib.backend} does not expose its acceleration structure")
+        n, root = C.c_uint32(), C.c_int32()
+        self._check(self.d.kjb_tlas_download_wide(self.ctx, C.byref(n), C.byref(root), None))
+        nodes = np.zeros((n.value, 32), np.uint32)
+        self._check(self.d.kjb_tlas_download_wide(self.ctx, C.byref(n), C.byref(root), nodes.ctypes.data))
+        return dict(nodes=nodes, root=int(root.value))
+
+    def trace_rays(self, rays, any_hit=False, cull_back=False, brute_force=False, binary=False):
         if not self.lib.has_tlas_trace:
             raise KjbError(f"{self.lib.backend} does not expose its acceleration structure")
         r = np.ascontiguousarray(rays, np.float32).reshape(-1, 8)
         out = np.zeros((len(r), 4), np.uint32)
-        flags = (1 if any_hit else 0) | (2 if cull_back else 0) | (4 if brute_force else 0)
+        flags = (1 if any_hit else 0) | (2 if cull_back else 0) | (4 if brute_force else 0) | (8 if binary else 0)
         self._check(self.d.kjb_tlas_trace(self.ctx, r.ctypes.data, len(r), flags, out.ctypes.data))
         return out
 
```
